# DakeQQ/Audio-Denoiser-ONNX

Measured on AMD Instinct MI355X. Metric: audio_seconds_per_second (GTCRN 16 kHz, batch=256 x 1 s chunks; RTF = 1/value), higher is better.
Workload: dtype f32; 1 GPU; GTCRN 16 kHz, batch=256 x 1 s chunks, fp32, int16 PCM in/out resident in HBM (BASELINE.json configs[1]); chunks_per_gpu=256, chunks_total=256, ranks=1, chunk_samples=16000, out_samples=15872, weights=seeded reference-architecture GTCRN (tests/golden/gtcrn_seed0.adew), stitch_all_gather=False

## Files before the change

### audio_denoiser_onnx_amd/csrc/ade_device.h

```cpp
#pragma once

#include "ade_internal.h"

namespace ade {
namespace dev {

__device__ __forceinline__ float fast_rcp(float x) { return __builtin_amdgcn_rcpf(x); }
__device__ __forceinline__ float fast_sqrt(float x) { return __builtin_amdgcn_sqrtf(x); }
__device__ __forceinline__ float fast_rsq(float x) { return __builtin_amdgcn_rsqf(x); }
__device__ __forceinline__ float sigmoid_f(float x) { return fast_rcp(1.0f + __expf(-x)); }
__device__ __forceinline__ float tanh_f(float x) {
    return 1.0f - 2.0f * fast_rcp(__expf(2.0f * x) + 1.0f);
}
__device__ __forceinline__ float prelu_f(float x, float a) { return x >= 0.0f ? x : a * x; }
__device__ __forceinline__ double shfl_xor_f64(double v, int mask) {
    union { double d; int i[2]; } u;
    u.d = v;
    u.i[0] = __shfl_xor(u.i[0], mask, 64);
    u.i[1] = __shfl_xor(u.i[1], mask, 64);
    return u.d;
}
__device__ __forceinline__ float prelu_sel(float a) { return a <= 1.0f ? __builtin_inff() : -__builtin_inff(); }
__device__ __forceinline__ float prelu_m(float x, float ax, float sel) { return __builtin_amdgcn_fmed3f(x, ax, sel); }

__device__ __forceinline__ void ld4(const float* p, float* v) {
    const float4 q = *reinterpret_cast<const float4*>(p);
    v[0] = q.x; v[1] = q.y; v[2] = q.z; v[3] = q.w;
}
__device__ __forceinline__ void ld8(const float* p, float* v) { ld4(p, v); ld4(p + 4, v + 4); }
__device__ __forceinline__ void ld16(const float* p, float* v) { ld8(p, v); ld8(p + 8, v + 8); }
__device__ __forceinline__ void st4(float* p, const float* v) {
    *reinterpret_cast<float4*>(p) = make_float4(v[0], v[1], v[2], v[3]);
}
__device__ __forceinline__ void st16(float* p, const float* v) { st4(p, v); st4(p + 4, v + 4); st4(p + 8, v + 8); st4(p + 12, v + 12); }

__device__ __forceinline__ void view_ld8_lo(const View& a, size_t pos, size_t frame, float* v) {
    ld8(a.x + pos * kCh, v);
    if (a.at) {
        float g[4];
        ld4(a.at + frame * 8, g);
#pragma unroll
        for (int i = 0; i < 4; ++i) v[2 * i] *= g[i];
    }
}
__device__ __forceinline__ void view_ld8_hi(const View& a, size_t pos, size_t frame, float* v) {
    ld8(a.x + pos * kCh + 8, v);
    if (a.at) {
        float g[4];
        ld4(a.at + frame * 8 + 4, g);
#pragma unroll
        for (int i = 0; i < 4; ++i) v[2 * i] *= g[i];
    }
}
__device__ __forceinline__ void view_ld16(const View& a, size_t pos, size_t frame, float* v) {
    view_ld8_lo(a, pos, frame, v);
    view_ld8_hi(a, pos, frame, v + 8);
}

template <int CTRL>
__device__ __forceinline__ float dpp_mov(float v) {
    return __int_as_float(__builtin_amdgcn_update_dpp(0, __float_as_int(v), CTRL, 0xF, 0xF, true));
}
template <int K> __device__ __forceinline__ float row_bcast(float v) { return dpp_mov<0x150 + K>(v); }
template <int K> __device__ __forceinline__ float quad_bcast(float v) { return dpp_mov<K * 0x55>(v); }
template <int N> __device__ __forceinline__ float row_ror(float v) { return dpp_mov<0x120 + N>(v); }
template <int N> __device__ __forceinline__ float quad_rot(float v) {
    return dpp_mov<((N) & 3) | (((N + 1) & 3) << 2) | (((N + 2) & 3) << 4) | (((N + 3) & 3) << 6)>(v);
}

struct Swapped { float a, b; };
__device__ __forceinline__ Swapped swap16(float v, float s) {
    const auto r = __builtin_amdgcn_permlane16_swap((unsigned)__float_as_int(v), (unsigned)__float_as_int(s), false, false);
    return Swapped{__int_as_float((int)r[0]), __int_as_float((int)r[1])};
}
__device__ __forceinline__ Swapped swap32(float v, float s) {
    const auto r = __builtin_amdgcn_permlane32_swap((unsigned)__float_as_int(v), (unsigned)__float_as_int(s), false, false);
    return Swapped{__int_as_float((int)r[0]), __int_as_float((int)r[1])};
}

template <int LANE> __device__ __forceinline__ float read_lane(float v) {
    return __int_as_float(__builtin_amdgcn_readlane(__float_as_int(v), LANE));
}
constexpr float kLog2e = 1.4426950408889634f;

#if defined(__clang__)
typedef float v4f __attribute__((ext_vector_type(4)));
#else
typedef float v4f __attribute__((vector_size(16)));
#endif
__device__ __forceinline__ v4f mfma16x16x4(float a, float b, v4f c) { return __builtin_amdgcn_mfma_f32_16x16x4f32(a, b, c, 0, 0, 0); }

#if defined(__clang__)
typedef float v2f __attribute__((ext_vector_type(2)));
#else
typedef float v2f __attribute__((vector_size(8)));
#endif
__device__ __forceinline__ v2f mk2(float a, float b) { v2f r; r[0] = a; r[1] = b; return r; }

#if defined(__has_attribute)
#if __has_attribute(address_space)
#define ADE_CONSTANT_AS __attribute__((address_space(4)))
#endif
#endif
#ifndef ADE_CONSTANT_AS
#define ADE_CONSTANT_AS
#endif
#if defined(__AMDGCN__)
#define ADE_KEEP_IN_LOOP(p) asm volatile("" : "+s"(p))
#else
#define ADE_KEEP_IN_LOOP(p) ((void)0)
#endif
#if defined(__AMDGCN__)
#define ADE_KEEP_AFTER(p, tok) asm volatile("" : "+s"(p), "+v"(tok))
#else
#define ADE_KEEP_AFTER(p, tok) ((void)0)
#endif
#if defined(__AMDGCN__)
#define ADE_SCALAR_COPY(dst, src) asm volatile("s_mov_b64 %0, %1" : "=s"(dst) : "s"(src))
#else
#define ADE_SCALAR_COPY(dst, src) ((dst) = (src))
#endif
#if defined(__AMDGCN__)
#define ADE_OPAQUE_V(x) asm volatile("" : "+v"(x))
#else
#define ADE_OPAQUE_V(x) ((void)0)
#endif
template <class T>
__device__ __forceinline__ T cload(const void ADE_CONSTANT_AS* p) {
    static_assert(sizeof(T) % 4 == 0, "dword-sized structs only");
    union U { T v; unsigned w[sizeof(T) / 4]; __device__ U() {} } u;
    const unsigned ADE_CONSTANT_AS* s = (const unsigned ADE_CONSTANT_AS*)p;
#pragma unroll
    for (size_t i = 0; i < sizeof(T) / 4; ++i) u.w[i] = s[i];
    return u.v;
}
typedef const float ADE_CONSTANT_AS* cfptr;
__device__ __forceinline__ cfptr cptr(const float* p) { return (cfptr)p; }

__device__ __forceinline__ void wave_sync() { __builtin_amdgcn_wave_barrier(); }
__device__ __forceinline__ float2 fcmul(float2 a, float2 b) { return make_float2(a.x * b.x - a.y * b.y, a.x * b.y + a.y * b.x); }
__device__ __forceinline__ void fradix4(float2* v) {
    const float2 a0 = make_float2(v[0].x + v[2].x, v[0].y + v[2].y);
    const float2 a1 = make_float2(v[0].x - v[2].x, v[0].y - v[2].y);
    const float2 a2 = make_float2(v[1].x + v[3].x, v[1].y + v[3].y);
    const float2 d = make_float2(v[1].x - v[3].x, v[1].y - v[3].y);
    const float2 a3 = make_float2(d.y, -d.x);
    v[0] = make_float2(a0.x + a2.x, a0.y + a2.y);
    v[1] = make_float2(a1.x + a3.x, a1.y + a3.y);
    v[2] = make_float2(a0.x - a2.x, a0.y - a2.y);
    v[3] = make_float2(a1.x - a3.x, a1.y - a3.y);
}
__device__ __forceinline__ void fft256_inplace(float2* v, float2* buf, int lane, const float2* __restrict__ tw256) {
    fradix4(v);
#pragma unroll
    for (int r = 0; r < 4; ++r) buf[4 * lane + r] = v[r];
    wave_sync();
#pragma unroll
    for (int pass = 1; pass < 4; ++pass) {
        const int Ns = 1 << (2 * pass);
        const int k = lane & (Ns - 1);
        const int tstride = 64 / Ns;
#pragma unroll
        for (int r = 0; r < 4; ++r) v[r] = buf[lane + 64 * r];
#pragma unroll
        for (int r = 1; r < 4; ++r) v[r] = fcmul(v[r], tw256[r * k * tstride]);
        fradix4(v);
        if (pass < 3) {
            wave_sync();
            const int j0 = ((lane - k) << 2) + k;
#pragma unroll
            for (int r = 0; r < 4; ++r) buf[j0 + r * Ns] = v[r];
            wave_sync();
        }
    }
}

__device__ __forceinline__ float4 keep4(bool ok, const float4& v) { return make_float4(ok ? v.x : 0.0f, ok ? v.y : 0.0f, ok ? v.z : 0.0f, ok ? v.w : 0.0f); }
__device__ __attribute__((aligned(16))) static float g_zero4[4] = {0.0f, 0.0f, 0.0f, 0.0f};
__device__ __forceinline__ float4 ld4_or_zero(bool ok, const float* p) { return *reinterpret_cast<const float4*>(ok ? p : g_zero4); }
__device__ __forceinline__ float4 pick4(bool first, const float4& a, const float4& b) {
    return make_float4(first ? a.x : b.x, first ? a.y : b.y, first ? a.z : b.z, first ? a.w : b.w);
}

#if defined(__AMDGCN__)
typedef unsigned ade_v4u __attribute__((ext_vector_type(4)));
__device__ __forceinline__ float4 xld4(const float* base, int float_off) {
    const __amdgpu_buffer_rsrc_t r = __builtin_amdgcn_make_buffer_rsrc(const_cast<float*>(base), 0, 0x7fffffff, 0x00020000);
    const ade_v4u v = __builtin_amdgcn_raw_buffer_load_b128(r, float_off * 4, 0, 16);
    return make_float4(__int_as_float((int)v.x), __int_as_float((int)v.y), __int_as_float((int)v.z), __int_as_float((int)v.w));
}
__device__ __forceinline__ void xst4(float* base, int float_off, const float4& v) {
    const __amdgpu_buffer_rsrc_t r = __builtin_amdgcn_make_buffer_rsrc(base, 0, 0x7fffffff, 0x00020000);
    ade_v4u u;
    u.x = (unsigned)__float_as_int(v.x); u.y = (unsigned)__float_as_int(v.y); u.z = (unsigned)__float_as_int(v.z); u.w = (unsigned)__float_as_int(v.w);
    __builtin_amdgcn_raw_buffer_store_b128(u, r, float_off * 4, 0, 16);
}
__device__ __forceinline__ float xld1(const float* p) { return __hip_atomic_load(p, __ATOMIC_RELAXED, __HIP_MEMORY_SCOPE_AGENT); }
__device__ __forceinline__ void xst1(float* p, float v) { __hip_atomic_store(p, v, __ATOMIC_RELAXED, __HIP_MEMORY_SCOPE_AGENT); }
__device__ __forceinline__ unsigned xflag_load(const unsigned* p) { return __hip_atomic_load(p, __ATOMIC_RELAXED, __HIP_MEMORY_SCOPE_AGENT); }
__device__ __forceinline__ void xflag_store(unsigned* p, unsigned v) { __hip_atomic_store(p, v, __ATOMIC_RELAXED, __HIP_MEMORY_SCOPE_AGENT); }
__device__ __forceinline__ void xdrain() { asm volatile("s_waitcnt vmcnt(0)" ::: "memory"); }
#else
__device__ __forceinline__ float4 xld4(const float* base, int float_off) { return *reinterpret_cast<const float4*>(base + float_off); }
__device__ __forceinline__ void xst4(float* base, int float_off, const float4& v) { *reinterpret_cast<float4*>(base + float_off) = v; }
__device__ __forceinline__ float xld1(const float* p) { return *p; }
__device__ __forceinline__ void xst1(float* p, float v) { *p = v; }
__device__ __forceinline__ unsigned xflag_load(const unsigned* p) { return *(const volatile unsigned*)p; }
__device__ __forceinline__ void xflag_store(unsigned* p, unsigned v) { *(volatile unsigned*)p = v; }
__device__ __forceinline__ void xdrain() {}
#endif
#if defined(__AMDGCN__)
__device__ __forceinline__ int xlimit() {
    const int ADE_CONSTANT_AS* p = (const int ADE_CONSTANT_AS*)__builtin_amdgcn_kernarg_segment_ptr();
    asm volatile("" : "+s"(p));
    return *p;
}
#else
__device__ __forceinline__ int xlimit() { return 20000000; }
#endif
__device__ __forceinline__ int xcode(int flag_index) { return (int)((blockIdx.x + 1u) << 4) | flag_index; }
__device__ __forceinline__ void xwait(unsigned* flag, int* err, int code) {
    if (xflag_load(flag) == 0u) {
        const long long t0 = wall_clock64();
        const int limit = xlimit();
        bool looked = false;
        do {
            __builtin_amdgcn_s_sleep(4);
            const long long dt = wall_clock64() - t0;
            if (dt > (limit >> 4) && !looked) {
                looked = true;
                if (*reinterpret_cast<volatile int*>(err) != 0) return;
            }
            if (dt > limit) {
                volatile int* const e = reinterpret_cast<volatile int*>(err);
                if (*e == 0) *e = code;
                return;
            }
        } while (xflag_load(flag) == 0u);
    }
    xflag_store(flag, 0u);
}

#if defined(__AMDGCN__)
__device__ __forceinline__ unsigned sys_load(const unsigned* p) { return __hip_atomic_load(p, __ATOMIC_RELAXED, __HIP_MEMORY_SCOPE_SYSTEM); }
__device__ __forceinline__ void sys_store(unsigned* p, unsigned v) { __hip_atomic_store(p, v, __ATOMIC_RELAXED, __HIP_MEMORY_SCOPE_SYSTEM); }
__device__ __forceinline__ void sys_acquire() { __builtin_amdgcn_fence(__ATOMIC_ACQUIRE, ""); }
__device__ __forceinline__ void sys_release() { __builtin_amdgcn_fence(__ATOMIC_RELEASE, ""); asm volatile("s_waitcnt vmcnt(0)" ::: "memory"); }
#else
__device__ __forceinline__ unsigned sys_load(const unsigned* p) { return *(const volatile unsigned*)p; }
__device__ __forceinline__ void sys_store(unsigned* p, unsigned v) { *(volatile unsigned*)p = v; }
__device__ __forceinline__ void sys_acquire() {}
__device__ __forceinline__ void sys_release() {}
#endif
__device__ __forceinline__ void wait_rows_in(const unsigned* ready, unsigned epoch, int* err, int code) {
    if (sys_load(ready) != epoch) {
        const long long t0 = wall_clock64();
        const int limit = xlimit();
        do {
            __builtin_amdgcn_s_sleep(8);
            if (wall_clock64() - t0 > limit) {
                volatile int* const e = reinterpret_cast<volatile int*>(err);
                if (*e == 0) *e = code;
                break;
            }
        } while (sys_load(ready) != epoch);
    }
    sys_acquire();
}
__device__ __forceinline__ void signal_rows_out(unsigned* count, unsigned* done, unsigned epoch, unsigned wgs) {
    sys_release();
#if defined(__AMDGCN__)
    const unsigned old = __hip_atomic_fetch_add(count, 1u, __ATOMIC_RELAXED, __HIP_MEMORY_SCOPE_AGENT);
#else
    const unsigned old = (*count)++;
#endif
    if (old + 1u == wgs) {
        xflag_store(count, 0u);
        sys_store(done, epoch);
    }
}

__device__ __forceinline__ void set_prio(int p) {
    if (p == 0) __builtin_amdgcn_s_setprio(0);
    else if (p == 1) __builtin_amdgcn_s_setprio(1);
    else if (p == 2) __builtin_amdgcn_s_setprio(2);
    else __builtin_amdgcn_s_setprio(3);
}

inline dim3 grid1(long long n, int per) { return dim3((unsigned)((n + per - 1) / per)); }

}
}
```

### audio_denoiser_onnx_amd/csrc/ade_engine.hip

```cpp
#include "ade_internal.h"
#include "ade_gtcrn_pack.h"

#include "../../include/ade.h"

#if !defined(HIPSIM)
#include <dlfcn.h>
#endif

#include <algorithm>
#include <cmath>
#include <cstdio>
#include <cstdlib>
#include <cstring>
#include <map>
#include <mutex>
#include <string>
#include <vector>

using namespace ade;

namespace {

thread_local std::string g_create_error;

// ... 311 lines not shown

ade_status build_device_constants(ade_engine* e) {
    Loader L{e};
    Arena A;
    const size_t o_win = A.alloc(kNfft), o_tw256 = A.alloc(512), o_tw512 = A.alloc(2 * 257 + 2), o_ws = A.alloc(kHop);
    {
        const float step = (float)(2.0 * M_PI / (double)kNfft);
        for (int n = 0; n < kNfft; ++n) A.f[o_win + n] = sqrtf(cosf((float)n * step) * -0.5f + 0.5f);
        for (int k = 0; k < 256; ++k) {
            A.f[o_tw256 + 2 * k] = (float)cos(2.0 * M_PI * k / 256.0);
            A.f[o_tw256 + 2 * k + 1] = (float)-sin(2.0 * M_PI * k / 256.0);
        }
        for (int k = 0; k <= 256; ++k) {
            A.f[o_tw512 + 2 * k] = (float)cos(2.0 * M_PI * k / 512.0);
            A.f[o_tw512 + 2 * k + 1] = (float)-sin(2.0 * M_PI * k / 512.0);
        }
        A.f[o_tw512 + 2 * 256] = -1.0f;
        A.f[o_tw512 + 2 * 256 + 1] = 0.0f;
        A.f[o_tw512 + 2 * 128] = 0.0f;
        A.f[o_tw256 + 2 * 64] = 0.0f;
        A.f[o_tw256 + 2 * 128 + 1] = 0.0f;
        A.f[o_tw256 + 2 * 192] = 0.0f;
        for (int r = 0; r < kHop; ++r) {
            const float a = A.f[o_win + r] * A.f[o_win + r], b = A.f[o_win + kHop + r] * A.f[o_win + kHop + r];
            A.f[o_ws + r] = a + b;
        }
    }
    const float* erb_t = L.get("erb.erb_weight_t", {kErbHigh, kErbBands});
    const float* ierb_t = L.get("erb.ierb_weight_t", {kErbBands, kErbHigh});
    if (L.st != ADE_OK) return L.st;
    std::vector<int> bm_start, bs_start;
    std::vector<float> bm_w, bs_w;
    int bm_count = 0, bs_count = 0;
    band_table(erb_t, kErbHigh, kErbBands, bm_start, bm_w, bm_count);
    band_table(ierb_t, kErbBands, kErbHigh, bs_start, bs_w, bs_count);
    const size_t o_bm = A.alloc(bm_w.size()), o_bs = A.alloc(bs_w.size());
    memcpy(&A.f[o_bm], bm_w.data(), bm_w.size() * 4);
    memcpy(&A.f[o_bs], bs_w.data(), bs_w.size() * 4);
    const float* w0 = L.get("encoder.en_convs.0.conv.weight", {16, 9, 1, 5});
    const float* b0 = L.get("encoder.en_convs.0.conv.bias", {16});
    const float* a0 = L.get("encoder.en_convs.0.act.weight", {1});
    const float* w1 = L.get("encoder.en_convs.1.conv.weight", {16, 8, 1, 5});
    const float* b1 = L.get("encoder.en_convs.1.conv.bias", {16});
    const float* a1 = L.get("encoder.en_convs.1.act.weight", {1});
    const float* w3 = L.get("decoder.de_convs.3.conv.weight", {16, 8, 1, 5});
    const float* b3 = L.get("decoder.de_convs.3.conv.bias", {16});
    const float* a3 = L.get("decoder.de_convs.3.act.weight", {1});
    const float* w4 = L.get("decoder.de_convs.4.conv.weight", {16, 2, 1, 5});
    const float* b4 = L.get("decoder.de_convs.4.conv.bias", {2});
    if (L.st != ADE_OK) return L.st;
    const size_t o_w0 = A.alloc(5 * 9 * 16 + 3 * 8 * 16), o_b0 = A.alloc(16), o_w1 = A.alloc(5 * 2 * 8 * 8), o_b1 = A.alloc(16);
    const size_t o_w3 = A.alloc(5 * 2 * 8 * 8), o_b3 = A.alloc(16), o_w4 = A.alloc(5 * 16 * 2), o_b4 = A.alloc(2);
    for (int co = 0; co < 16; ++co)
        for (int ci = 0; ci < 9; ++ci)
            for (int k = 0; k < 5; ++k) A.f[o_w0 + (k * 9 + ci) * 16 + co] = w0[(co * 9 + ci) * 5 + k];
    for (int co = 0; co < 16; ++co)
        for (int c = 0; c < 3; ++c) {
            for (int jj = 0; jj < 7; ++jj) {
                float sum = 0.0f;
                for (int k = 0; k < 5; ++k) {
                    const int o = jj - k;
                    if (o >= 0 && o < 3) sum += w0[(co * 9 + c * 3 + o) * 5 + k];
                }
                A.f[o_w0 + 720 + (c * 8 + jj) * 16 + co] = sum;
            }
            A.f[o_w0 + 720 + (c * 8 + 7) * 16 + co] = -w0[(co * 9 + c * 3 + 2) * 5 + 1];
        }
    for (int g = 0; g < 2; ++g)
        for (int co = 0; co < 8; ++co)
            for (int ci = 0; ci < 8; ++ci)
                for (int k = 0; k < 5; ++k) {
                    A.f[o_w1 + ((k * 2 + g) * 8 + ci) * 8 + co] = w1[((g * 8 + co) * 8 + ci) * 5 + k];
                    A.f[o_w3 + ((k * 2 + g) * 8 + ci) * 8 + co] = w3[((g * 8 + ci) * 8 + co) * 5 + k];
                }
    for (int ci = 0; ci < 16; ++ci)
        for (int co = 0; co < 2; ++co)
            for (int k = 0; k < 5; ++k) A.f[o_w4 + (k * 16 + ci) * 2 + co] = w4[(ci * 2 + co) * 5 + k];
    memcpy(&A.f[o_b0], b0, 64);
    memcpy(&A.f[o_b1], b1, 64);
    memcpy(&A.f[o_b3], b3, 64);
    memcpy(&A.f[o_b4], b4, 8);
    GtOff gte[3], gtd[3];
    DpOff dpo[2];
    static const int en_dil[3] = {1, 2, 5}, de_dil[3] = {5, 2, 1};
    for (int i = 0; i < 3; ++i) {
        if (!load_gt(L, A, "encoder.en_convs." + std::to_string(i + 2) + ".", false, gte[i])) return L.st;
        if (!load_gt(L, A, "decoder.de_convs." + std::to_string(i) + ".", true, gtd[i])) return L.st;
    }
    if (!load_dp(L, A, "dpgrnn1.", dpo[0]) || !load_dp(L, A, "dpgrnn2.", dpo[1])) return L.st;

    HIP_TRY(e, hipMalloc((void**)&e->d_weights, A.f.size() * sizeof(float)));
    HIP_TRY(e, hipMemcpy(e->d_weights, A.f.data(), A.f.size() * sizeof(float), hipMemcpyHostToDevice));
    std::vector<int> ints(bm_start);
    ints.insert(ints.end(), bs_start.begin(), bs_start.end());
    HIP_TRY(e, hipMalloc((void**)&e->d_ints, ints.size() * sizeof(int)));
    HIP_TRY(e, hipMalloc((void**)&e->d_clk, kClkSlots * sizeof(long long)));
    HIP_TRY(e, hipMemset(e->d_clk, 0, kClkSlots * sizeof(long long)));
    HIP_TRY(e, hipMemcpy(e->d_ints, ints.data(), ints.size() * sizeof(int), hipMemcpyHostToDevice));
    const float* W = e->d_weights;
    e->tabs.win = W + o_win;
    e->tabs.tw256 = reinterpret_cast<const float2*>(W + o_tw256);
    e->tabs.tw512 = reinterpret_cast<const float2*>(W + o_tw512);
    e->tabs.win_sum = W + o_ws;
    e->erb_bm = BandTab{e->d_ints, W + o_bm, bm_count, kErbBands};
    e->erb_bs = BandTab{e->d_ints + kErbBands, W + o_bs, bs_count, kErbHigh};
    e->en0 = ConvW{W + o_w0, W + o_b0, a0[0]};
    e->en1 = ConvW{W + o_w1, W + o_b1, a1[0]};
    e->de3 = ConvW{W + o_w3, W + o_b3, a3[0]};
    e->de4 = ConvW{W + o_w4, W + o_b4, 0.0f};
    for (int i = 0; i < 3; ++i) {
        const GtOff* src[2] = {&gte[i], &gtd[i]};
        GtConvW* dst[2] = {&e->en_gt[i], &e->de_gt[i]};
        for (int k = 0; k < 2; ++k) {
            const GtOff& o = *src[k];
            *dst[k] = GtConvW{W + o.pw1, W + o.pw1_b, W + o.dw, W + o.dw_b, W + o.pw2, W + o.pw2_b, W + o.gru, W + o.fc,
                              o.s1, o.s2, k == 0 ? en_dil[i] : de_dil[i], W + o.tra_rot};
        }
    }
    for (int i = 0; i < 2; ++i) {
        const DpOff& o = dpo[i];
        e->dp[i] = DpW{W + o.intra_gru, W + o.inter_gru, W + o.fc[0], W + o.fc_b[0], W + o.ln_w[0], W + o.ln_b[0],
                       W + o.fc[1], W + o.fc_b[1], W + o.ln_w[1], W + o.ln_b[1], W + o.inter_rot};
    }
    return ADE_OK;
}

void free_graphs(ade_engine* e) {
    for (auto& g : e->graphs) {
        if (g.exec) hipGraphExecDestroy(g.exec);
        if (g.graph) hipGraphDestroy(g.graph);
    }
    e->graphs.clear();
}

void free_exchange(ade_engine* e) {
    if (e->d_xchg) hipFree(e->d_xchg);
    if (e->d_xflags) hipFree(e->d_xflags);
    e->d_xchg = nullptr; e->d_xflags = nullptr;
    e->xchg_capacity = 0; e->xchg_segments = 0;
}

void free_workspace(ade_engine* e) {
    free_graphs(e);
    if (e->ws) hipFree(e->ws);
    if (e->d_pcm_in) hipFree(e->d_pcm_in);
    if (e->d_pcm_out) hipFree(e->d_pcm_out);
    if (e->d_f32_out) hipFree(e->d_f32_out);
    if (e->h_pcm_in) hipHostFree(e->h_pcm_in);
    if (e->h_pcm_out) hipHostFree(e->h_pcm_out);
    if (e->h_f32_out) hipHostFree(e->h_f32_out);
    if (e->rs_in) hipFree(e->rs_in);
    if (e->rs_out) hipFree(e->rs_out);
    if (e->d_fixed) hipFree(e->d_fixed);
    e->d_fixed = nullptr;
    free_exchange(e);
    for (float** p : {&e->gt_tmp, &e->gt_in, &e->gt_wave, &e->gt_mean, &e->d_f32_in}) { if (*p) hipFree(*p); *p = nullptr; }
    for (uint16_t** p : {&e->d_f16_in, &e->d_f16_out}) { if (*p) hipFree(*p); *p = nullptr; }
    for (uint16_t** p : {&e->h_f16_in, &e->h_f16_out}) { if (*p) hipHostFree(*p); *p = nullptr; }
    e->f16_capacity = 0;
    e->rs_in = e->rs_out = nullptr;
    e->ws = nullptr;
    e->d_pcm_in = e->d_pcm_out = nullptr;
    e->d_f32_out = nullptr;
    e->h_pcm_in = e->h_pcm_out = nullptr;
    e->h_f32_out = nullptr;
    e->capacity = 0;
}

int pick_geometry(const ade_engine* e, int B);

ade_status ensure_exchange(ade_engine* e) {
    if (e->sub) return ADE_OK;
    if (!e->d_xerr) {
        HIP_TRY(e, hipHostMalloc((void**)&e->d_xerr, kXErrWords * sizeof(int), hipHostMallocDefault));
        for (int k = 0; k < kXErrWords; ++k) e->d_xerr[k] = 0;
    }
    int nseg = 0;
    if (e->use_fused && !e->gt_sand) {
        const int g = pick_geometry(e, e->capacity);
        if (g >= 0) nseg = fused_segments(e->T, g);
    }
    if (nseg <= 1) nseg = 0;
    if (nseg == e->xchg_segments && (nseg == 0 || e->xchg_capacity >= e->capacity)) return ADE_OK;
    if (e->d_xchg && nseg <= e->xchg_segments && e->xchg_capacity >= e->capacity) return ADE_OK;
    if (e->stream) HIP_TRY(e, hipStreamSynchronize(e->stream));
    free_graphs(e);
    free_exchange(e);
    if (nseg) {
        const size_t B = (size_t)e->capacity;
        HIP_TRY(e, hipMalloc((void**)&e->d_xchg, B * nseg * (size_t)kXFloats * sizeof(float)));
        HIP_TRY(e, hipMalloc((void**)&e->d_xflags, B * nseg * (size_t)kXFlags * sizeof(unsigned)));
        HIP_TRY(e, hipMemset(e->d_xflags, 0, B * nseg * (size_t)kXFlags * sizeof(unsigned)));
        e->xchg_capacity = e->capacity;
    }
    e->xchg_segments = nseg;
    return ADE_OK;
}

ade_status reserve(ade_engine* e, int batch) {
    if (batch <= e->capacity) return ensure_exchange(e);
    HIP_TRY(e, hipSetDevice(e->device));
    if (e->stream) HIP_TRY(e, hipStreamSynchronize(e->stream));
    free_workspace(e);
    const size_t B = (size_t)batch, T = (size_t)e->T;
    if (e->sub) {
        std::string derr;
        const int rc = e->sub->reserve(batch, derr);
        if (rc != ADE_OK) return fail(e, (ade_status)rc, derr);
        HIP_TRY(e, hipMalloc((void**)&e->d_pcm_in, B * e->in_len * sizeof(int16_t)));
        HIP_TRY(e, hipMalloc((void**)&e->d_pcm_out, B * e->out_len * sizeof(int16_t)));
        HIP_TRY(e, hipMalloc((void**)&e->d_f32_out, B * e->out_len * sizeof(float)));
        HIP_TRY(e, hipHostMalloc((void**)&e->h_pcm_in, B * e->in_len * sizeof(int16_t), hipHostMallocDefault));
        HIP_TRY(e, hipHostMalloc((void**)&e->h_pcm_out, B * e->out_len * sizeof(int16_t), hipHostMallocDefault));
        HIP_TRY(e, hipHostMalloc((void**)&e->h_f32_out, B * e->out_len * sizeof(float), hipHostMallocDefault));
        if (e->resample) {
            HIP_TRY(e, hipMalloc((void**)&e->rs_in, B * e->channels * e->rs_model_in * sizeof(float)));
            HIP_TRY(e, hipMalloc((void**)&e->rs_out, B * e->out_channels * e->n_outputs * e->rs_model_out * sizeof(float)));
        }
        if (e->gt_float_in) HIP_TRY(e, hipMalloc((void**)&e->d_f32_in, B * (size_t)e->in_len * sizeof(float)));
        e->capacity = batch;
        return ADE_OK;
    }
    const size_t nfr = B * T;
    struct Carve { float** p; size_t n; };
    std::vector<Carve> cs = {
        {&e->mean, B}, {&e->spec, nfr * 2 * kBinsPad}, {&e->feat, nfr * 3 * kErbPad}, {&e->e0, nfr * kF1 * kCh},
        {&e->e1, nfr * kFw * kCh}, {&e->h, nfr * kFw * kCh}, {&e->zt, nfr * 8}, {&e->rnn, nfr * kFw * kCh},
        {&e->d3, nfr * kF1 * kCh}, {&e->mask, nfr * 2 * kErbPad}, {&e->frames, nfr * kNfft}};
    for (int i = 0; i < 3; ++i) {
        cs.push_back({&e->xe[i], nfr * kFw * kCh});
        cs.push_back({&e->ate[i], nfr * 8});
        cs.push_back({&e->xd[i], nfr * kFw * kCh});
        cs.push_back({&e->atd[i], nfr * 8});
    }
    for (int i = 0; i < 2; ++i) {
        cs.push_back({&e->dpm[i], nfr * kFw * kCh});
        cs.push_back({&e->dpo[i], nfr * kFw * kCh});
    }
    size_t total = 0;
    for (auto& c : cs) total += (c.n + 63) & ~(size_t)63;
    HIP_TRY(e, hipMalloc((void**)&e->ws, total * sizeof(float)));
    size_t off = 0;
    for (auto& c : cs) {
        *c.p = e->ws + off;
        off += (c.n + 63) & ~(size_t)63;
    }
    HIP_TRY(e, hipMalloc((void**)&e->d_pcm_in, B * e->in_len * sizeof(int16_t)));
    HIP_TRY(e, hipMalloc((void**)&e->d_pcm_out, B * e->out_len * sizeof(int16_t)));
    HIP_TRY(e, hipMalloc((void**)&e->d_f32_out, B * e->out_len * sizeof(float)));
    HIP_TRY(e, hipHostMalloc((void**)&e->h_pcm_in, B * e->in_len * sizeof(int16_t), hipHostMallocDefault));
    HIP_TRY(e, hipHostMalloc((void**)&e->h_pcm_out, B * e->out_len * sizeof(int16_t), hipHostMallocDefault));
    HIP_TRY(e, hipHostMalloc((void**)&e->h_f32_out, B * e->out_len * sizeof(float), hipHostMallocDefault));
    {
        ChunkFixed F{};
        F.tabs = e->tabs; F.erb_bm = e->erb_bm; F.erb_bs = e->erb_bs;
        F.en0 = e->en0; F.en1 = e->en1; F.de3 = e->de3; F.de4 = e->de4;
        for (int i = 0; i < 3; ++i) { F.en_gt[i] = e->en_gt[i]; F.de_gt[i] = e->de_gt[i]; F.xe[i] = e->xe[i]; F.xd[i] = e->xd[i]; }
        for (int i = 0; i < 2; ++i) { F.dp[i] = e->dp[i]; F.dpo[i] = e->dpo[i]; }
        F.spec = e->spec; F.e0 = e->e0; F.e1 = e->e1;
        HIP_TRY(e, hipMalloc((void**)&e->d_fixed, sizeof(ChunkFixed)));
        HIP_TRY(e, hipMemcpy(e->d_fixed, &F, sizeof(ChunkFixed), hipMemcpyHostToDevice));
    }
    if (e->gt_sand) {
        HIP_TRY(e, hipMalloc((void**)&e->gt_tmp, B * (size_t)e->gt_l1 * sizeof(float)));
        HIP_TRY(e, hipMalloc((void**)&e->gt_in, B * (size_t)e->gt_lm * sizeof(float)));
        HIP_TRY(e, hipMalloc((void**)&e->gt_wave, B * (size_t)e->gt_keep * sizeof(float)));
        HIP_TRY(e, hipMalloc((void**)&e->gt_mean, B * sizeof(float)));
        if (e->gt_float_in) HIP_TRY(e, hipMalloc((void**)&e->d_f32_in, B * (size_t)e->in_len * sizeof(float)));
    }
    e->capacity = batch;
    return ensure_exchange(e);
}

struct Seq {
    ade_engine* e;
    hipStream_t s;
    bool prof;
    int cursor = 0;
    void begin(const char* name) {
        if (!prof) return;
        int si = -1;
        for (size_t i = 0; i < e->stats.size(); ++i)
            if (e->stats[i].name == name) si = (int)i;
        if (si < 0) { e->stats.push_back(KernelStat{name, 0.f, 0}); si = (int)e->stats.size() - 1; }
        if ((int)e->events.size() <= cursor) {
            hipEvent_t a, b;
            hipEventCreate(&a);
            hipEventCreate(&b);
            e->events.push_back({a, b});
            e->event_stat.push_back(si);
        }
        e->event_stat[cursor] = si;
        hipEventRecord(e->events[cursor].first, s);
    }
    void end() {
        if (!prof) return;
        hipEventRecord(e->events[cursor].second, s);
        ++cursor;
        e->events_used = cursor;
    }
};

int pick_geometry(const ade_engine* e, int ) {
    if (e->geometry >= 0) return fused_supported(e->T, e->geometry) ? e->geometry : -1;
    for (int g = fused_geometries() - 1; g >= 0; --g)
        if (fused_supported(e->T, g)) return g;
    return -1;
}

void enqueue(ade_engine* e, hipStream_t s, const int16_t* d_in, int B, int16_t* d_out, float* d_f32, bool prof) {
    const int T = e->T, nfr = B * T;
    Seq q{e, s, prof};
    const View none{nullptr, nullptr};
    const int geo = pick_geometry(e, B);
    const bool fused = e->use_fused && geo >= 0 && !e->gt_sand;
    e->last_fused = fused;
    View x{e->e1, nullptr};
    if (fused) {
        SegPlan plan{};
        plan.nseg = fused_segments(T, geo); plan.xchg = e->d_xchg; plan.flags = e->d_xflags; plan.err = e->d_xerr; plan.wave_swap = e->wave_swap;
        plan.prio = e->seg_prio;
        plan.withhold = e->xchg_withhold;
        plan.wait_ticks = e->xwait_ticks;
        e->last_geometry = geo;
        long long* clk = prof ? e->d_clk : nullptr;
        if (clk) (void)hipMemsetAsync(e->d_clk, 0, kClkSlots * sizeof(long long), s);
        const float* dc = nullptr;
        if (e->n_win > 1) {
            q.begin("pcm_mean"); launch_pcm_mean(s, d_in, B, e->in_len, e->mean, e->n_win); q.end();
            dc = e->mean;
        }
        if (e->use_single && (!prof || e->profile_mode >= 2)) {
            ChunkCall C{};
            C.fixed = e->d_fixed;
            C.dc = dc;
            C.stagger = (geo == 0 && B >= 192) ? e->stagger_ticks : 0;
            C.pcm_in = d_in; C.pcm_out = d_out; C.f32_out = d_f32; C.L = e->in_len; C.T = T; C.B = B;
            C.plan = plan;
            C.full_taps = e->full_taps;
            C.clk = (prof && e->profile_mode == 3) ? e->d_clk : nullptr;
            q.begin("gtcrn_chunk"); launch_gtcrn_chunk(s, geo, C); q.end();
            return;
        }
        q.begin("front"); launch_front(s, geo, plan, d_in, B, e->in_len, T, e->tabs, e->erb_bm, e->en0, e->en1, e->spec, e->e0, e->e1, clk, dc); q.end();
        for (int i = 0; i < 3; ++i) {
            q.begin("gtblock"); launch_gtblock(s, geo, plan, i, x.x, nullptr, e->en_gt[i], e->xe[i], B, T, (prof && i == 0) ? e->d_clk : nullptr); q.end();
            x = View{e->xe[i], nullptr};
        }
        for (int i = 0; i < 2; ++i) {
            q.begin("dpgrnn"); launch_dpgrnn(s, geo, plan, i, x.x, e->dp[i], e->dpo[i], B, T, (prof && i == 0) ? e->d_clk : nullptr); q.end();
            x = View{e->dpo[i], nullptr};
        }
        for (int i = 0; i < 3; ++i) {
            q.begin("gtblock"); launch_gtblock(s, geo, plan, 3 + i, x.x, e->xe[2 - i], e->de_gt[i], e->xd[i], B, T, nullptr); q.end();
            x = View{e->xd[i], nullptr};
        }
        q.begin("back"); launch_back(s, geo, plan, x.x, e->e1, e->e0, e->spec, e->de3, e->de4, e->erb_bs, e->tabs, d_out, d_f32, B, T, clk); q.end();
        return;
    }
    if (e->gt_sand) {
        q.begin("sandwich_in");
        launch_gt_sandwich_in(s, e->cur_fin ? nullptr : d_in, e->cur_fin, B / e->n_win, e->in_len * e->n_win, e->gt_l1 * e->n_win, e->gt_lm * e->n_win, e->gt_lerp1,
                              e->gt_lerp2, e->gt_gain, e->gt_tmp, e->gt_mean, e->gt_in);
        q.end();
        q.begin("stft_feat"); launch_stft_pcm(s, nullptr, nullptr, B, e->gt_lm, T, e->tabs, e->erb_bm, e->spec, e->feat, true, e->gt_in); q.end();
    } else {
        q.begin("pcm_mean"); launch_pcm_mean(s, d_in, B, e->in_len, e->mean, e->n_win); q.end();
        q.begin("stft_feat"); launch_stft_pcm(s, d_in, e->mean, B, e->in_len, T, e->tabs, e->erb_bm, e->spec, e->feat); q.end();
    }
    q.begin("conv0"); launch_conv0(s, e->feat, e->en0, e->e0, nfr); q.end();
    q.begin("conv1"); launch_conv1(s, e->e0, e->en1, e->e1, nfr); q.end();
    for (int i = 0; i < 3; ++i) {
        q.begin("gt_pw1"); launch_gt_pw1(s, x, none, e->en_gt[i], e->h, nfr); q.end();
        q.begin("gt_dw_pw2"); launch_gt_dw_pw2(s, e->h, x, none, e->en_gt[i], e->xe[i], e->zt, B, T); q.end();
        q.begin("tra_gru"); launch_tra(s, e->zt, e->en_gt[i], e->ate[i], B, T); q.end();
        x = View{e->xe[i], e->ate[i]};
    }
    for (int i = 0; i < 2; ++i) {
        q.begin("intra_gru"); launch_intra_gru(s, x, e->dp[i].intra_gru, e->rnn, nfr); q.end();
        q.begin("fc_ln_res"); launch_fc_ln_res(s, e->rnn, x, e->dp[i].intra_fc, e->dp[i].intra_fc_b, e->dp[i].intra_ln_w,
                                               e->dp[i].intra_ln_b, e->dpm[i], B, T); q.end();
        q.begin("inter_gru"); launch_inter_gru(s, e->dpm[i], e->dp[i].inter_gru, e->rnn, B, T, nullptr, e->dp[i].inter_rot); q.end();
        q.begin("fc_ln_res"); launch_fc_ln_res(s, e->rnn, View{e->dpm[i], nullptr}, e->dp[i].inter_fc, e->dp[i].inter_fc_b,
                                               e->dp[i].inter_ln_w, e->dp[i].inter_ln_b, e->dpo[i], B, T); q.end();
        x = View{e->dpo[i], nullptr};
    }
    for (int i = 0; i < 3; ++i) {
        const View skip{e->xe[2 - i], e->ate[2 - i]};
        q.begin("gt_pw1"); launch_gt_pw1(s, x, skip, e->de_gt[i], e->h, nfr); q.end();
        q.begin("gt_dw_pw2"); launch_gt_dw_pw2(s, e->h, x, skip, e->de_gt[i], e->xd[i], e->zt, B, T); q.end();
        q.begin("tra_gru"); launch_tra(s, e->zt, e->de_gt[i], e->atd[i], B, T); q.end();
        x = View{e->xd[i], e->atd[i]};
    }
    q.begin("deconv3"); launch_deconv3(s, x, View{e->e1, nullptr}, e->de3, e->d3, nfr); q.end();
    q.begin("deconv4"); launch_deconv4(s, e->d3, e->e0, e->de4, e->mask, nfr); q.end();
    q.begin("istft_mask"); launch_istft_masked(s, e->spec, e->mask, e->erb_bs, e->tabs, e->frames, nfr); q.end();
    if (e->gt_sand) {
        q.begin("sandwich_out");
        launch_gt_sandwich_out(s, e->frames, e->tabs, B, T, e->gt_keep, e->gt_wave, d_out, d_f32, e->out_len, e->gt_lerp_out, e->gt_scale_first);
        q.end();
        return;
    }
    q.begin("ola_pcm"); launch_ola_pcm(s, e->frames, e->tabs, B, T, d_out, d_f32); q.end();
}

ade_status run(ade_engine* e, hipStream_t s, const int16_t* d_in, int B, int16_t* d_out, float* d_f32) {
    if (B == 0) return ADE_OK;
    e->last_batch = B;
    std::string sub_err;
    int sub_rc = ADE_OK;
    auto launch_all = [&](bool timed) {
        if (e->sub && e->resample) {
            const long long rows_in = (long long)B * e->channels, rows_out = (long long)B * e->out_channels * e->n_outputs;
            if (e->cur_fin) launch_resample_in_f32(s, e->cur_fin, e->rs_in, rows_in, e->in_len / e->channels, e->rs_model_in, e->rs_scale_in, e->rs_in_gain);
            else launch_resample_in(s, d_in, e->rs_in, rows_in, e->in_len / e->channels, e->rs_model_in, e->rs_scale_in);
            e->sub->float_in = e->rs_in;
            e->sub->float_src = e->cur_fin;
            e->sub->float_src_gain = e->rs_in_gain;
            sub_rc = e->sub->run(s, d_in, B, nullptr, e->rs_out, sub_err);
            e->sub->float_in = nullptr;
            e->sub->float_src = nullptr;
            if (e->rs_sandwich_out)
                launch_gt_out(s, e->rs_out, d_out, d_f32, rows_out, e->rs_model_out, e->out_len / (e->out_channels * e->n_outputs), e->rs_scale_out, e->rs_scale_first,
                              e->rs_nan_to_num);
            else
                launch_resample_out(s, e->rs_out, d_out, d_f32, rows_out, e->rs_model_out, e->out_len / (e->out_channels * e->n_outputs), e->rs_scale_out,
                                    e->rs_pcm_scale, e->rs_truncate_i32, e->rs_f32_scale, e->rs_nan_to_num);
        } else if (e->sub) sub_rc = e->sub->run(s, d_in, B, d_out, d_f32, sub_err);
        else enqueue(e, s, d_in, B, d_out, d_f32, timed);
    };
    if (e->sub && (e->profile || !e->use_graph || !e->graph_supported)) {
        launch_all(false);
        return sub_rc == ADE_OK ? ADE_OK : fail(e, (ade_status)sub_rc, sub_err);
    }
    if (e->profile) {
        for (auto& st : e->stats) { st.ms = 0.f; st.launches = 0; }
        e->events_used = 0;
        enqueue(e, s, d_in, B, d_out, d_f32, true);
        HIP_TRY(e, hipStreamSynchronize(s));
        for (size_t i = 0; i < (size_t)e->events_used; ++i) {
            float ms = 0.f;
            hipEventElapsedTime(&ms, e->events[i].first, e->events[i].second);
            e->stats[e->event_stat[i]].ms += ms;
            e->stats[e->event_stat[i]].launches += 1;
        }
        return ADE_OK;
    }
    const bool one_kernel = !e->sub && e->use_fused && e->use_single && pick_geometry(e, B) >= 0 && !e->gt_sand;
    if (e->use_graph && e->graph_supported && !one_kernel) {
        GraphEntry* hit = nullptr;
        for (auto& g : e->graphs)
            if (g.in == d_in && g.out_pcm == d_out && g.out_f32 == d_f32 && g.batch == B) hit = &g;
        if (!hit) {
            if (hipStreamBeginCapture(s, hipStreamCaptureModeThreadLocal) == hipSuccess) {
                launch_all(false);
                hipGraph_t graph = nullptr;
                hipGraphExec_t exec = nullptr;
                if (hipStreamEndCapture(s, &graph) == hipSuccess && graph && sub_rc == ADE_OK &&
                    hipGraphInstantiate(&exec, graph, nullptr, nullptr, 0) == hipSuccess) {
                    if (e->graphs.size() >= 8) {
                        hipGraphExecDestroy(e->graphs.front().exec);
                        hipGraphDestroy(e->graphs.front().graph);
                        e->graphs.erase(e->graphs.begin());
                    }
                    e->graphs.push_back(GraphEntry{d_in, d_out, d_f32, B, exec, graph});
                    hit = &e->graphs.back();
                } else {
                    if (graph) hipGraphDestroy(graph);
                    e->graph_supported = false;
                }
            } else {
                (void)hipGetLastError();
                e->graph_supported = false;
            }
        }
        if (hit) {
            HIP_TRY(e, hipGraphLaunch(hit->exec, s));
            return ADE_OK;
        }
    }
    launch_all(false);
    if (sub_rc != ADE_OK) return fail(e, (ade_status)sub_rc, sub_err);
    HIP_TRY(e, hipGetLastError());
    return ADE_OK;
}

const char* xflag_name(int idx) {
    return idx < kXFlagTra ? "depthwise-convolution history" : (idx < kXFlagInter ? "TRA state" : (idx < kXFlagOla ? "inter-frame GRU state" : "overlap-add carry"));
}
ade_status exchange_status(ade_engine* h, const char* who, bool earlier) {
    if (h->sub) {
        const int code = h->sub->exchange_error_and_reset();
        if (code) {
            h->timed_out = true;
            char msg[320];
            snprintf(msg, sizeof msg, "%s: %s: a segment hand-off (%s) of the fused network stages timed out (%.1f ms)%s; the call's output is not valid "
                     "(ADE_HG_FUSED=0 runs the multi-kernel sequence, option xwait_ms raises the bound)", who, "sub-engine", xflag_name(code & 15), h->xwait_ticks * 1e-5,
                     earlier ? " in an earlier call on a caller-provided stream" : "");
            return fail(h, ADE_ERR_DEVICE, msg);
        }
    }
    if (!h->d_xerr) return ADE_OK;
    int code = 0, word = 0;
    for (int k = 0; k < kXErrWords && !code; ++k) { code = ((volatile int*)h->d_xerr)[k]; word = k; }
    if (!code) return ADE_OK;
    (void)hipDeviceSynchronize();
    for (int k = 0; k < kXErrWords; ++k) h->d_xerr[k] = 0;
    if (h->d_xflags) (void)hipMemset(h->d_xflags, 0, (size_t)h->xchg_capacity * h->xchg_segments * kXFlags * sizeof(unsigned));
    const int block = (code >> 4) - 1, idx = code & 15, B = h->xl_B[word] > 0 ? h->xl_B[word] : (h->last_batch > 0 ? h->last_batch : 1), chunk0 = h->xl_B[word] > 0 ? h->xl_chunk0[word] : 0;
    h->timed_out = true;
    char msg[384];
    if (idx == 15)
        snprintf(msg, sizeof msg, "%s: fused path%s: segment %d of chunk %d timed out (%.1f ms) waiting for its rows of the host batch to be copied in; no output was produced "
                 "(option host_stream=1 copies the batch before the launch, option xwait_ms raises the bound)",
                 who, earlier ? " (an earlier call on a caller-provided stream)" : "", block / B, chunk0 + block % B, h->xwait_ticks * 1e-5);
    else
        snprintf(msg, sizeof msg,
                 "%s: fused path%s: segment %d of chunk %d timed out (%.1f ms) waiting for the %s of its predecessor workgroup; no output was produced "
                 "(option geometry=0 runs whole chunks per workgroup, option xwait_ms raises the bound)",
                 who, earlier ? " (an earlier call on a caller-provided stream)" : "", block / B, chunk0 + block % B, h->xwait_ticks * 1e-5, xflag_name(idx));
    return fail(h, ADE_ERR_DEVICE, msg);
}

}

struct ade_stream {
    ade_engine* e = nullptr;
    int device = 0;
    int S = 0, N = 0;
    bool first = true, flushed = false;
    void* sub_state = nullptr;
    int in_ch = 1, delay = kHop;
    int16_t *pcm_prev = nullptr, *pcm_hist = nullptr, *concat = nullptr, *d_in = nullptr, *d_out = nullptr, *h_in = nullptr, *h_out = nullptr;
    float *d_f32 = nullptr, *h_f32 = nullptr;
    float* state = nullptr;
    size_t state_floats = 0;
    float* dc = nullptr;
    float* hist[6][2] = {};
    int hist_cur[6] = {};
    float* tra_h[6] = {};
    float* inter_h[2] = {};
    float* carry = nullptr;
    bool fused = false;
    int geo = -1, geo_flush = -1;
    ade::ChunkFixed* d_fixed = nullptr;
    float* xq = nullptr;
    unsigned* xq_flags = nullptr;
    float* xstate[2] = {};
    unsigned* xstate_flags[2] = {};
    int xcur = 0;
    int* xerr = nullptr;
    float* ws = nullptr;
    float *spec = nullptr, *feat = nullptr, *e0 = nullptr, *e1 = nullptr, *h = nullptr, *zt = nullptr, *rnn = nullptr, *d3 = nullptr, *mask = nullptr,
          *frames = nullptr, *xe[3] = {}, *ate[3] = {}, *xd[3] = {}, *atd[3] = {}, *dpm[2] = {}, *dpo[2] = {};
};

namespace {

void enqueue_stream(ade_stream* st, hipStream_t s, const int16_t* d_in, int16_t* d_out, float* d_f32, bool flush = false) {
    ade_engine* e = st->e;
    const int B = st->S, T = flush ? 1 : st->N, nfr = B * T, P = T * kHop;
    if (flush) launch_stream_concat_flush(s, st->pcm_hist, st->pcm_prev, st->concat, B);
    else {
        launch_stream_concat(s, st->pcm_hist, d_in, st->concat, B, P, st->first);
        launch_stream_keep(s, st->concat, st->pcm_hist, st->pcm_prev, B, P);
    }
    if (st->fused) {
        const int geo = flush ? st->geo_flush : st->geo;
        ChunkCall C{};
        C.fixed = st->d_fixed;
        C.pcm_in = st->concat; C.pcm_out = d_out; C.f32_out = d_f32; C.dc = st->dc;
        C.L = P + kHop; C.T = T; C.B = B;
        SegPlan plan{};
        plan.nseg = fused_segments(T, geo);
        plan.xchg = st->xq; plan.flags = st->xq_flags; plan.err = st->xerr;
        plan.wait_ticks = e->xwait_ticks;
        plan.carry_in = st->first ? nullptr : st->xstate[st->xcur];
        plan.carry_in_flags = st->first ? nullptr : st->xstate_flags[st->xcur];
        plan.carry_out = st->xstate[st->xcur ^ 1];
        plan.carry_out_flags = st->xstate_flags[st->xcur ^ 1];
        plan.stream = 1;
        C.plan = plan;
        launch_gtcrn_chunk(s, geo, C);
        st->xcur ^= 1;
        st->first = false;
        return;
    }
    launch_stft_pcm(s, st->concat, st->dc, B, P + kHop, T, e->tabs, e->erb_bm, st->spec, st->feat, false);
    launch_conv0(s, st->feat, e->en0, st->e0, nfr);
    launch_conv1(s, st->e0, e->en1, st->e1, nfr);
    const View none{nullptr, nullptr};
    View x{st->e1, nullptr};
    auto gt_block = [&](int gi, const GtConvW& w, View in, View skip, float* xn, float* at) {
        launch_gt_pw1(s, in, skip, w, st->h, nfr);
        const int cur = st->hist_cur[gi];
        launch_gt_dw_pw2(s, st->h, in, skip, w, xn, st->zt, B, T, st->hist[gi][cur]);
        launch_hist_shift(s, st->hist[gi][cur], st->h, st->hist[gi][cur ^ 1], B, T, 2 * w.dilation);
        st->hist_cur[gi] = cur ^ 1;
        launch_tra(s, st->zt, w, at, B, T, st->tra_h[gi]);
    };
    for (int i = 0; i < 3; ++i) {
        gt_block(i, e->en_gt[i], x, none, st->xe[i], st->ate[i]);
        x = View{st->xe[i], st->ate[i]};
    }
    for (int i = 0; i < 2; ++i) {
        launch_intra_gru(s, x, e->dp[i].intra_gru, st->rnn, nfr);
// ... 1465 lines not shown
```

### audio_denoiser_onnx_amd/csrc/ade_stage_frontback.h

```cpp
#pragma once
#include "ade_stage_net.h"

namespace ade {
namespace stage {

constexpr int kWbuf = 264;
constexpr size_t kTabFloats = 512 + 2 * 256 + 2 * 264;
constexpr int kBmCap = 16;
constexpr int kBsCap = 4;

__device__ __forceinline__ float2 rfft_bin(float2 zk, float2 zp, float2 w) {
    const float2 e = make_float2(0.5f * (zk.x + zp.x), 0.5f * (zk.y - zp.y));
    const float2 d = make_float2(0.5f * (zk.x - zp.x), 0.5f * (zk.y + zp.y));
    const float2 o = make_float2(d.y, -d.x);
    return make_float2(e.x + (w.x * o.x - w.y * o.y), e.y + (w.x * o.y + w.y * o.x));
}

struct LdsTabs { const float* win; const float2* tw256; const float2* tw512; };
template <class G>
__device__ __forceinline__ LdsTabs stage_tables(float* dst, const FftTabs& t, int tid) {
    constexpr int kFusedThreads = G::kThreads;
    float* win = dst;
    float* tw256 = dst + 512;
    float* tw512 = tw256 + 512;
    for (int i = tid; i < 512; i += kFusedThreads) { win[i] = t.win[i]; tw256[i] = reinterpret_cast<const float*>(t.tw256)[i]; }
    for (int i = tid; i < 514; i += kFusedThreads) tw512[i] = reinterpret_cast<const float*>(t.tw512)[i];
    return LdsTabs{win, reinterpret_cast<const float2*>(tw256), reinterpret_cast<const float2*>(tw512)};
}

__device__ __forceinline__ void load_frame_pairs(const int16_t* __restrict__ row, int L, int t, int lane, bool live, bool pair_ok, int* raw, int centre = kNfft / 2) {
#pragma unroll
    for (int r = 0; r < 4; ++r) {
        const int n = lane + 64 * r;
        const int j0 = kHop * t + 2 * n - centre;
        if (!live) {
            raw[r] = 0;
        } else if (pair_ok && j0 >= 0 && j0 + 1 < L) {
            raw[r] = *reinterpret_cast<const int*>(row + j0);
        } else {
            int ja = j0, jb = j0 + 1;
            ja = ja < 0 ? -ja : (ja >= L ? 2 * (L - 1) - ja : ja);
            jb = jb < 0 ? -jb : (jb >= L ? 2 * (L - 1) - jb : jb);
            raw[r] = ((int)row[ja] & 0xffff) | ((int)row[jb] << 16);
        }
    }
}

__device__ __forceinline__ void erb_merge(const float* wtab, int count, int s0, const float2* buf, int lane, float* fr) {
    float a0 = 0.0f, a1 = 0.0f, a2 = 0.0f;
    for (int n = 0; n < count; ++n) {
        const float wv = wtab[n * kErbBands + lane];
        const float2 x = buf[kErbLow + min(s0 + n, kErbHigh - 1)];
        a0 += fast_sqrt((x.x * x.x + x.y * x.y) + 1e-12f) * wv;
        a1 += x.x * wv;
        a2 += x.y * wv;
    }
    fr[kErbLow + lane] = a0;
    fr[kErb + kErbLow + lane] = a1;
    fr[2 * kErb + kErbLow + lane] = a2;
}

constexpr int kC0TailW = 27 * 16;
constexpr int kC1TailW = 3 * 2 * 64;
template <class G> constexpr size_t front_smem_bytes() {
    return ((size_t)G::kTileF * kWbuf * 2 + (size_t)G::kTileF * 3 * kErb + (size_t)4 * G::kTileF * kF1 * 4 + kTabFloats +
            (size_t)(G::kLean ? 0 : kBmCap) * kErbBands + kC0TailW + kC1TailW + 16) * 4;
}

template <class G>
__device__ __forceinline__ void front_stage(float* smem, int chunk, const Seg& sg, const int16_t* __restrict__ pcm, int L, const FftTabs& tabs,
                                            const BandTab& erb, const ConvW& c0, const ConvW& c1, float* __restrict__ spec,
                                            float* __restrict__ e0, float* __restrict__ e1, long long* __restrict__ clk,
                                            const float* __restrict__ dc_rows = nullptr) {
    constexpr int kFusedThreads = G::kThreads, kTileF = G::kTileF, kTileP1 = kTileF * kF1;
    constexpr size_t kFrontFeatFloats = (size_t)kTileF * 3 * kErb;
    constexpr int kGroupShift = (kFusedThreads == 1024 ? 9 : (kFusedThreads == 512 ? 8 : 7));
    static_assert(kFusedThreads == 1024 || kFusedThreads == 512 || kFusedThreads == 256, "front / back conv rounds: 64 lanes per frame");
    constexpr int kBmRows = G::kLean ? 0 : kBmCap;
    const int T = sg.T, tbeg = sg.t0, tend = sg.t0 + sg.nT;
    float2* wbuf_all = reinterpret_cast<float2*>(smem);
    float* feat = smem + kTileF * kWbuf * 2;
    float4* E0 = reinterpret_cast<float4*>(feat + kFrontFeatFloats);
    float* E0f = reinterpret_cast<float*>(E0);
    float* tabmem = reinterpret_cast<float*>(E0 + 4 * kTileP1);
    float* erbw = tabmem + kTabFloats;
    float* w0t = erbw + kBmRows * kErbBands;
    float* w1t = w0t + kC0TailW;
    int* red = reinterpret_cast<int*>(w1t + kC1TailW);
    int tid_ = threadIdx.x;
    ADE_OPAQUE_V(tid_);
    const int tid = tid_, wave = tid >> 6, lane = tid & 63;
    const int16_t* row = pcm + (size_t)chunk * L;
    const int P0 = T * kF1, P = T * kFw;
    float* e0c = e0 + (size_t)chunk * kCh * P0;
    float* e1c = e1 + (size_t)chunk * kCh * P;
    float* specc = spec + (size_t)chunk * T * 2 * kBinsPad;
    ADE_CLK(32);
    const bool pair_ok = ((L & 1) == 0) && ((reinterpret_cast<size_t>(row) & 3) == 0);
    int raw[4];
    const int centre = sg.stream ? 0 : kNfft / 2;
    load_frame_pairs(row, L, tbeg + wave, lane, tbeg + wave < tend, pair_ok, raw, centre);
    const LdsTabs lt = stage_tables<G>(tabmem, tabs, tid);
    const bool erb_lds = erb.count <= kBmRows;
    if (erb_lds)
        for (int i = tid; i < erb.count * kErbBands; i += kFusedThreads) erbw[i] = erb.w[i];
    const int erb_s0 = erb.start[lane];
    for (int i = tid; i < kC0TailW; i += kFusedThreads) w0t[i] = c0.w[i];
    for (int i = tid; i < kC1TailW; i += kFusedThreads) w1t[i] = c1.w[i];
    const float b0t = c0.b[tid & 15], b1t = c1.b[tid & 15];

    if (!dc_rows) {
        int s = 0;
        if (((L & 7) == 0) && ((reinterpret_cast<size_t>(row) & 15) == 0)) {
            const int4* r4 = reinterpret_cast<const int4*>(row);
#pragma unroll 2
            for (int i = tid; i < (L >> 3); i += kFusedThreads) {
                const int4 q = r4[i];
                s += (int)(short)(q.x & 0xffff) + (q.x >> 16) + (int)(short)(q.y & 0xffff) + (q.y >> 16)
                   + (int)(short)(q.z & 0xffff) + (q.z >> 16) + (int)(short)(q.w & 0xffff) + (q.w >> 16);
            }
        } else {
            for (int i = tid; i < L; i += kFusedThreads) s += (int)row[i];
        }
#pragma unroll
        for (int off = 32; off >= 1; off >>= 1) s += __shfl_xor(s, off);
        if (lane == 0) red[wave] = s;
    }
    __syncthreads();
    float dc;
    if (dc_rows) {
        dc = dc_rows[chunk];
    } else {
        long long tot = 0;
#pragma unroll
        for (int i = 0; i < kTileF; ++i) tot += red[i];
        dc = (float)((double)tot / ((double)L * 32768.0));
    }
    ADE_CLK(33);
    long long clk_prev = ADE_CLK_START();
    const cfptr c0b = cptr(c0.b), c1b = cptr(c1.b);
    const cfptr c0e = cptr(c0.w) + 5 * 9 * 16;

    for (int t0 = tbeg; t0 < tend; t0 += kTileF) {
        const int nf = tend - t0 < kTileF ? tend - t0 : kTileF;
        {
            int tq = tid;
            ADE_OPAQUE_V(tq);
            const int wave = tq >> 6, lane = tq & 63;
            float2* buf = wbuf_all + wave * kWbuf;
            const int t = t0 + wave;
            const bool live = wave < nf;
            float2 v[4];
#pragma unroll
            for (int r = 0; r < 4; ++r) {
                const int n = lane + 64 * r;
                const float sa = (float)(short)(raw[r] & 0xffff) * (1.0f / 32768.0f) - dc;
                const float sb = (float)(raw[r] >> 16) * (1.0f / 32768.0f) - dc;
                v[r] = make_float2(sa * lt.win[2 * n], sb * lt.win[2 * n + 1]);
            }
            {
                const int tn = t + kTileF;
                load_frame_pairs(row, L, tn, lane, tn < tend, pair_ok, raw, centre);
            }
            fft256_inplace(v, buf, lane, lt.tw256);
            wave_sync();
#pragma unroll
            for (int r = 0; r < 4; ++r) buf[lane + 64 * r] = v[r];
            wave_sync();
            {
                float2 xa[2], xb[2];
#pragma unroll
                for (int r = 0; r < 2; ++r) {
                    const int k = lane + 64 * r;
                    const float2 zk = buf[k], zp = buf[(256 - k) & 255];
                    xa[r] = rfft_bin(zk, zp, lt.tw512[k]);
                    xb[r] = rfft_bin(zp, zk, lt.tw512[256 - k]);
                }
                float2 xm = make_float2(0.0f, 0.0f);
                if (lane == 0) { const float2 z = buf[128]; xm = rfft_bin(z, z, lt.tw512[128]); }
                wave_sync();
#pragma unroll
                for (int r = 0; r < 2; ++r) {
                    const int k = lane + 64 * r;
                    buf[k] = xa[r];
                    buf[256 - k] = xb[r];
                }
                if (lane == 0) buf[128] = xm;
            }
            wave_sync();
            if (live) {
                float* fr = feat + (size_t)wave * 3 * kErb;
#pragma unroll
                for (int r = 0; r < 5; ++r) {
                    if (r == 4 && lane != 0) break;
                    const int k = r < 4 ? lane + 64 * r : 256;
                    const float2 x = buf[k];
                    specc[((size_t)t * 2 + 0) * kBinsPad + k] = x.x;
                    specc[((size_t)t * 2 + 1) * kBinsPad + k] = x.y;
                    if (k < kErbLow) {
                        fr[k] = fast_sqrt((x.x * x.x + x.y * x.y) + 1e-12f);
                        fr[kErb + k] = x.x;
                        fr[2 * kErb + k] = x.y;
                    }
                }
                if (erb_lds) erb_merge(erbw, erb.count, erb_s0, buf, lane, fr);
                else erb_merge(erb.w, erb.count, erb_s0, buf, lane, fr);
            }
        }
        __syncthreads();
        ADE_CLK(34);
        ADE_CLK_ACC(40);
        {
            int tq = tid;
            ADE_OPAQUE_V(tq);
            const int tl = tq >> 6, g = (tq >> 4) & 3, j = tq & 15;
            if (tl < nf) {
                const float* fr = feat + (size_t)tl * 3 * kErb;
                float wa[6];
#pragma unroll
                for (int kk = 0; kk < 6; ++kk) wa[kk] = c0e[((kk >> 1) * 8 + 4 * (kk & 1) + g) * 16 + j];
                v4f cb;
#pragma unroll
                for (int r = 0; r < 4; ++r) cb[r] = c0b[4 * g + r];
                const float sel0 = prelu_sel(c0.slope);
#pragma unroll
                for (int mt = 0; mt < 4; ++mt) {
                    const int fo = 16 * mt + j;
                    const int q0 = 2 * fo - 3 + g;
                    const bool v0 = q0 >= 0;
                    const int q1 = g == 3 ? 0 : 2 * fo + 1 + g;
                    const bool v1 = g == 3 ? fo == 0 : q1 < kErb;
                    v4f d = cb;
#pragma unroll
                    for (int c = 0; c < 3; ++c) {
                        const float x0 = fr[c * kErb + q0], x1 = fr[c * kErb + q1];
                        d = mfma16x16x4(wa[2 * c], v0 ? x0 : 0.0f, d);
                        d = mfma16x16x4(wa[2 * c + 1], v1 ? x1 : 0.0f, d);
                    }
                    const float4 r4 = make_float4(prelu_m(d[0], d[0] * c0.slope, sel0), prelu_m(d[1], d[1] * c0.slope, sel0),
                                                  prelu_m(d[2], d[2] * c0.slope, sel0), prelu_m(d[3], d[3] * c0.slope, sel0));
                    const int idx = tl * kF1 + fo;
                    E0[g * kTileP1 + idx] = r4;
                    *reinterpret_cast<float4*>(e0c + ((size_t)g * P0 + (size_t)t0 * kF1 + idx) * 4) = r4;
                }
            }
        }
        if (tid < kTileF * 16) {
            int tq = tid;
            ADE_OPAQUE_V(tq);
            const int tl = tq >> 4, co = tq & 15;
            if (tl < nf) {
                const float* fr = feat + (size_t)tl * 3 * kErb;
                float acc = b0t;
#pragma unroll
                for (int k = 0; k < 3; ++k)
#pragma unroll
                    for (int c = 0; c < 3; ++c)
#pragma unroll
                        for (int o = 0; o < 3; ++o) {
                            const int q = 2 * (kF1 - 1) - 3 + k + o;
                            const float x = q < kErb ? fr[c * kErb + q] : 0.0f;
                            acc += w0t[(k * 9 + c * 3 + o) * 16 + co] * x;
                        }
                acc = prelu_f(acc, c0.slope);
                const int idx = tl * kF1 + (kF1 - 1);
                E0f[((size_t)(co >> 2) * kTileP1 + idx) * 4 + (co & 3)] = acc;
                e0c[((size_t)(co >> 2) * P0 + t0 * kF1 + idx) * 4 + (co & 3)] = acc;
            }
        }
        __syncthreads();
        ADE_CLK(35);
        ADE_CLK_ACC(41);
        {
            int tq = tid;
            ADE_OPAQUE_V(tq);
            const int g = __builtin_amdgcn_readfirstlane(tq >> kGroupShift);
            const int tl = (tq >> 5) & (kTileF - 1), fo = tq & 31;
            if (tl < nf) {
                cfptr cw = cptr(c1.w);
                ADE_KEEP_IN_LOOP(cw);
                float acc[8];
#pragma unroll
                for (int co = 0; co < 8; ++co) acc[co] = c1b[g * 8 + co];
#pragma unroll
                for (int k = 0; k < 5; ++k) {
                    const int fi = 2 * fo - 2 + k;
                    const bool ok = fi >= 0;
                    const int pp = tl * kF1 + (ok ? fi : 0);
                    const float4 xa = E0[(2 * g) * kTileP1 + pp], xb = E0[(2 * g + 1) * kTileP1 + pp];
                    const float x[8] = {ok ? xa.x : 0.0f, ok ? xa.y : 0.0f, ok ? xa.z : 0.0f, ok ? xa.w : 0.0f,
                                        ok ? xb.x : 0.0f, ok ? xb.y : 0.0f, ok ? xb.z : 0.0f, ok ? xb.w : 0.0f};
#pragma unroll
                    for (int ci = 0; ci < 8; ++ci)
#pragma unroll
                        for (int co = 0; co < 8; ++co) acc[co] += cw[((k * 2 + g) * 8 + ci) * 8 + co] * x[ci];
                }
#pragma unroll
                for (int co = 0; co < 8; ++co) acc[co] = prelu_f(acc[co], c1.slope);
                const int p = t0 * kFw + tl * kFw + fo;
                st4(e1c + ((size_t)(2 * g) * P + p) * 4, acc);
                st4(e1c + ((size_t)(2 * g + 1) * P + p) * 4, acc + 4);
            }
        }
        if (tid < kTileF * 16) {
            int tq = tid;
            ADE_OPAQUE_V(tq);
            const int tl = tq >> 4, g = (tq >> 3) & 1, co = tq & 7;
            if (tl < nf) {
                float acc = b1t;
#pragma unroll
                for (int k = 0; k < 3; ++k) {
                    const int pp = tl * kF1 + (kF1 - 3) + k;
#pragma unroll
                    for (int ci = 0; ci < 8; ++ci)
                        acc += w1t[((k * 2 + g) * 8 + ci) * 8 + co] * E0f[((size_t)(2 * g + (ci >> 2)) * kTileP1 + pp) * 4 + (ci & 3)];
                }
                acc = prelu_f(acc, c1.slope);
                const int p = t0 * kFw + tl * kFw + (kFw - 1);
                e1c[((size_t)(2 * g + (co >> 2)) * P + p) * 4 + (co & 3)] = acc;
            }
        }
        ADE_CLK(36);
        ADE_CLK_ACC(42);
    }
}

constexpr int kC3TailW = 2 * 2 * 64;
constexpr int kC4TailW = 2 * 16 * 2;
template <class G> constexpr size_t back_smem_bytes() {
    return ((size_t)4 * G::kTileF * kFw * 4 + (size_t)4 * G::kTileF * kF1 * 4 + (size_t)G::kTileF * 2 * kErbPad + (size_t)kHop + kTabFloats + (size_t)kBsCap * kErbHigh +
            kC3TailW + kC4TailW + (G::kLean ? 0 : kHop + kErbHigh + kHop)) * 4;
}

template <class G>
__device__ __forceinline__ void back_stage(float* smem, int chunk, const Seg& sg, const float* __restrict__ x, const float* __restrict__ e1,
                                           const float* __restrict__ e0, const float* __restrict__ spec, const ConvW& c3, const ConvW& c4,
                                           const BandTab& bs, const FftTabs& tabs, int16_t* __restrict__ pcm,
                                           float* __restrict__ f32, long long* __restrict__ clk) {
    constexpr int kFusedThreads = G::kThreads, kTileF = G::kTileF, kTileP1 = kTileF * kF1, kTileP = kTileF * kFw;
    constexpr size_t kBackAccFloats = (size_t)kNfft + (size_t)kHop * (kTileF - 1);
    static_assert((size_t)4 * kTileP * 4 >= (size_t)kTileF * kWbuf * 2, "the S tile must be able to hold the FFT buffers");
    static_assert((size_t)4 * kTileP1 * 4 >= kBackAccFloats, "the D tile must be able to hold the overlap-add accumulator");
    constexpr int kSUnits = 4 * kTileP;
    constexpr int kSThreads = kSUnits / 3;
    static_assert(kSThreads * 3 == kSUnits && kSThreads <= kFusedThreads, "S staging split");
    constexpr int kGroupShift = (kFusedThreads == 1024 ? 9 : (kFusedThreads == 512 ? 8 : 7));
    constexpr bool kLean = G::kLean;
    const int T = sg.T, tbeg = sg.t0, tend = sg.t0 + sg.nT;
    float4* S = reinterpret_cast<float4*>(smem);
    float* Sf = smem;
    float2* wbuf_all = reinterpret_cast<float2*>(smem);
    float4* D = S + 4 * kTileP;
    float* Df = reinterpret_cast<float*>(D);
    float* M = reinterpret_cast<float*>(D + 4 * kTileP1);
    float* acc = Df;
    float* cbuf = M + kTileF * 2 * kErbPad;
    float* tabmem = cbuf + kHop;
    float* bsw = tabmem + kTabFloats;
    float* w3t = bsw + kBsCap * kErbHigh;
    float* w4t = w3t + kC3TailW;
    float* wsum = kLean ? const_cast<float*>(tabs.win_sum) : w4t + kC4TailW;
    int* bss = reinterpret_cast<int*>(wsum + kHop);
    float* pend = kLean ? sg.xo + kXPendOff : reinterpret_cast<float*>(bss + kErbHigh);
    int tid_ = threadIdx.x;
    ADE_OPAQUE_V(tid_);
    const int tid = tid_;
    const int P0 = T * kF1, P = T * kFw;
    const float* xc = x + (size_t)chunk * kCh * P;
    const float* e1c = e1 + (size_t)chunk * kCh * P;
    const float* e0c = e0 + (size_t)chunk * kCh * P0;
    const float* specc = spec + (size_t)chunk * T * 2 * kBinsPad;
    const int trim = sg.stream ? 0 : kHop;
    const int out_len = sg.stream ? kHop * T : kHop * (T - 1);
    int16_t* po = pcm ? pcm + (size_t)chunk * out_len : nullptr;
    float* fo32 = f32 ? f32 + (size_t)chunk * out_len : nullptr;
    ADE_CLK(48);

    auto issue_s = [&](int t0n, bool go, float4* sa, float4* sb) {
        const int nfn = tend - t0n < kTileF ? tend - t0n : kTileF;
        int tq = tid;
        ADE_OPAQUE_V(tq);
        const bool on = go && tq < kSThreads;
#pragma unroll
        for (int i = 0; i < 3; ++i) {
            const int u = tq + kSThreads * i, q = u / kTileP, idx = u - q * kTileP;
            const int idc = idx < nfn * kFw ? idx : 0;
            const size_t off = ((size_t)q * P + (size_t)t0n * kFw + idc) * 4;
            sa[i] = on ? *reinterpret_cast<const float4*>(xc + off) : make_float4(0.0f, 0.0f, 0.0f, 0.0f);
            sb[i] = on ? *reinterpret_cast<const float4*>(e1c + off) : make_float4(0.0f, 0.0f, 0.0f, 0.0f);
        }
    };
    auto commit_s = [&](const float4* sa, const float4* sb) {
        int tq = tid;
        ADE_OPAQUE_V(tq);
        if (tq < kSThreads) {
#pragma unroll
            for (int i = 0; i < 3; ++i)
                S[tq + kSThreads * i] = make_float4(sa[i].x + sb[i].x, sa[i].y + sb[i].y, sa[i].z + sb[i].z, sa[i].w + sb[i].w);
        }
    };
    auto issue_e0 = [&](int t0n, bool go, float4* ea, float4* eb) {
        const int nfn = tend - t0n < kTileF ? tend - t0n : kTileF;
        int tq = tid;
        ADE_OPAQUE_V(tq);
        const int g = tq >> kGroupShift, tl = (tq >> 5) & (kTileF - 1), m = tq & 31;
        const bool on = go && tl < nfn;
        const int pe = on ? tl * kF1 + 2 * m : 0;
#pragma unroll
        for (int h = 0; h < 2; ++h) {
            const float* src = e0c + ((size_t)(2 * g + h) * P0 + (size_t)t0n * kF1 + pe) * 4;
            ea[h] = on ? *reinterpret_cast<const float4*>(src) : make_float4(0.0f, 0.0f, 0.0f, 0.0f);
            eb[h] = on ? *reinterpret_cast<const float4*>(src + 4) : make_float4(0.0f, 0.0f, 0.0f, 0.0f);
        }
    };
    float4 sa0[3], sb0[3];
    issue_s(tbeg, true, sa0, sb0);
    float4 ea[2], eb[2];
    issue_e0(tbeg, true, ea, eb);
    const LdsTabs lt = stage_tables<G>(tabmem, tabs, tid);
    if (!kLean)
        for (int i = tid; i < kHop; i += kFusedThreads) wsum[i] = tabs.win_sum[i];
    const bool bs_lds = bs.count <= kBsCap;
    int bs_s[4] = {0, 0, 0, 0};
    if (bs_lds) {
        for (int i = tid; i < bs.count * kErbHigh; i += kFusedThreads) bsw[i] = bs.w[i];
        if (!kLean) {
            for (int i = tid; i < kErbHigh; i += kFusedThreads) bss[i] = bs.start[i];
        } else {
            int tq = tid;
            ADE_OPAQUE_V(tq);
            const int lane = tq & 63;
#pragma unroll
            for (int r = 1; r < 5; ++r) {
                const int k = r < 4 ? lane + 64 * r : 256;
                bs_s[r - 1] = (k >= kErbLow && (r < 4 || lane == 0)) ? bs.start[k - kErbLow] : 0;
            }
        }
    }
    for (int i = tid; i < kC3TailW; i += kFusedThreads) w3t[i] = c3.w[(i < 128 ? 2 : 4) * 128 + (i & 127)];
    for (int i = tid; i < kC4TailW; i += kFusedThreads) w4t[i] = c4.w[(i < 32 ? 2 : 4) * 32 + (i & 31)];
    const float b3t = c3.b[tid & 15], b4t = c4.b[tid & 1];
    for (int i = tid; i < kHop; i += kFusedThreads) cbuf[i] = 0.0f;
    const cfptr c3b = cptr(c3.b), c4b = cptr(c4.b), c4w = cptr(c4.w);
    commit_s(sa0, sb0);
    long long clk_prev = ADE_CLK_START();

    for (int t0 = tbeg; t0 < tend; t0 += kTileF) {
        const int nf = tend - t0 < kTileF ? tend - t0 : kTileF;
        float sre[5], sim[5];
        float wsr[4] = {1.0f, 1.0f, 1.0f, 1.0f};
        if (kLean) ld4(wsum + ((tid * 4) & (kHop - 1)), wsr);
        {
            int tq = tid;
            ADE_OPAQUE_V(tq);
            const int wave = tq >> 6, lane = tq & 63;
            const int tcp = wave < nf ? t0 + wave : t0;
#pragma unroll
            for (int r = 0; r < 5; ++r) {
                const int k = r < 4 ? lane + 64 * r : 256;
                sre[r] = (r < 4 || lane == 0) ? specc[((size_t)tcp * 2 + 0) * kBinsPad + k] : 0.0f;
                sim[r] = (r < 4 || lane == 0) ? specc[((size_t)tcp * 2 + 1) * kBinsPad + k] : 0.0f;
            }
        }
        __syncthreads();
        ADE_CLK(49);
        ADE_CLK_ACC(56);
        {
            int tq = tid;
            ADE_OPAQUE_V(tq);
            const int g = __builtin_amdgcn_readfirstlane(tq >> kGroupShift);
            const int tl = (tq >> 5) & (kTileF - 1), m = tq & 31;
            if (tl < nf) {
                const int idx = tl * kFw + m, pe = tl * kF1 + 2 * m;
                cfptr cw = cptr(c3.w);
                ADE_KEEP_IN_LOOP(cw);
                float ev[8], od[8];
#pragma unroll
                for (int co = 0; co < 8; ++co) { ev[co] = c3b[g * 8 + co]; od[co] = c3b[g * 8 + co]; }
#pragma unroll
                for (int dlt = -1; dlt <= 1; ++dlt) {
                    const bool ok = m + dlt >= 0;
                    const int ke = 2 - 2 * dlt, ko = 3 - 2 * dlt;
                    const int ps = idx + (ok ? dlt : 0);
                    const float4 xa = S[(2 * g) * kTileP + ps], xb = S[(2 * g + 1) * kTileP + ps];
                    const float xv[8] = {ok ? xa.x : 0.0f, ok ? xa.y : 0.0f, ok ? xa.z : 0.0f, ok ? xa.w : 0.0f,
                                         ok ? xb.x : 0.0f, ok ? xb.y : 0.0f, ok ? xb.z : 0.0f, ok ? xb.w : 0.0f};
#pragma unroll
                    for (int ci = 0; ci < 8; ++ci)
#pragma unroll
                        for (int co = 0; co < 8; ++co) {
                            ev[co] += cw[((ke * 2 + g) * 8 + ci) * 8 + co] * xv[ci];
                            if (dlt >= 0) od[co] += cw[((ko * 2 + g) * 8 + ci) * 8 + co] * xv[ci];
                        }
                }
#pragma unroll
                for (int h = 0; h < 2; ++h) {
                    D[(2 * g + h) * kTileP1 + pe] =
                        make_float4(prelu_f(ev[4 * h], c3.slope) + ea[h].x, prelu_f(ev[4 * h + 1], c3.slope) + ea[h].y,
                                    prelu_f(ev[4 * h + 2], c3.slope) + ea[h].z, prelu_f(ev[4 * h + 3], c3.slope) + ea[h].w);
                    D[(2 * g + h) * kTileP1 + pe + 1] =
                        make_float4(prelu_f(od[4 * h], c3.slope) + eb[h].x, prelu_f(od[4 * h + 1], c3.slope) + eb[h].y,
                                    prelu_f(od[4 * h + 2], c3.slope) + eb[h].z, prelu_f(od[4 * h + 3], c3.slope) + eb[h].w);
                }
            }
        }
        if (tid < kTileF * 16) {
            int tq = tid;
            ADE_OPAQUE_V(tq);
            const int tl = tq >> 4, g = (tq >> 3) & 1, co = tq & 7;
            if (tl < nf) {
                const int pe = tl * kF1 + (kF1 - 1);
                const float eadd = e0c[((size_t)(2 * g + (co >> 2)) * P0 + (size_t)t0 * kF1 + pe) * 4 + (co & 3)];
                float ev = b3t;
#pragma unroll
                for (int dlt = -1; dlt <= 0; ++dlt) {
                    const int ps = tl * kFw + (kFw - 1) + dlt;
#pragma unroll
                    for (int ci = 0; ci < 8; ++ci)
                        ev += w3t[(dlt < 0 ? 128 : 0) + (g * 8 + ci) * 8 + co] * Sf[((size_t)(2 * g + (ci >> 2)) * kTileP + ps) * 4 + (ci & 3)];
                }
                Df[((size_t)(2 * g + (co >> 2)) * kTileP1 + pe) * 4 + (co & 3)] = prelu_f(ev, c3.slope) + eadd;
            }
        }
        __syncthreads();
        ADE_CLK(50);
        ADE_CLK_ACC(57);
        float4 sa[3], sb[3];
        const bool has_next = t0 + kTileF < tend;
        issue_s(has_next ? t0 + kTileF : t0, has_next, sa, sb);
        issue_e0(has_next ? t0 + kTileF : t0, has_next, ea, eb);
        {
            int tq = tid;
            ADE_OPAQUE_V(tq);
            const int tl = tq >> 6, m = tq & 63;
            if (tl < nf) {
                const int idx = tl * kF1 + m;
                v2f ev = mk2(c4b[0], c4b[1]), od = ev;
#pragma unroll
                for (int dlt = -1; dlt <= 1; ++dlt) {
                    const bool ok = m + dlt >= 0;
                    const int ke = 2 - 2 * dlt, ko = 3 - 2 * dlt;
#pragma unroll
                    for (int q = 0; q < 4; ++q) {
                        const float4 xq = D[q * kTileP1 + idx + (ok ? dlt : 0)];
                        const float xv[4] = {ok ? xq.x : 0.0f, ok ? xq.y : 0.0f, ok ? xq.z : 0.0f, ok ? xq.w : 0.0f};
#pragma unroll
                        for (int c = 0; c < 4; ++c) {
                            ev += mk2(c4w[(ke * 16 + 4 * q + c) * 2], c4w[(ke * 16 + 4 * q + c) * 2 + 1]) * xv[c];
                            if (dlt >= 0) od += mk2(c4w[(ko * 16 + 4 * q + c) * 2], c4w[(ko * 16 + 4 * q + c) * 2 + 1]) * xv[c];
                        }
                    }
                }
                float* mr = M + (size_t)tl * 2 * kErbPad;
#pragma unroll
                for (int co = 0; co < 2; ++co) {
                    mr[co * kErbPad + 2 * m] = tanh_f(ev[co]);
                    mr[co * kErbPad + 2 * m + 1] = tanh_f(od[co]);
                }
            }
        }
        if (tid < kTileF * 2) {
            const int tl = tid >> 1, co = tid & 1;
            if (tl < nf) {
                float ev = b4t;
#pragma unroll
                for (int dlt = -1; dlt <= 0; ++dlt) {
                    const int ps = tl * kF1 + (kF1 - 1) + dlt;
#pragma unroll
                    for (int ci = 0; ci < 16; ++ci)
                        ev += w4t[(dlt < 0 ? 32 : 0) + ci * 2 + co] * Df[((size_t)(ci >> 2) * kTileP1 + ps) * 4 + (ci & 3)];
                }
                M[(size_t)tl * 2 * kErbPad + co * kErbPad + (kErb - 1)] = tanh_f(ev);
            }
        }
        __syncthreads();
        ADE_CLK(51);
        ADE_CLK_ACC(58);
        {
            int tq = tid;
            ADE_OPAQUE_V(tq);
            const int wave = tq >> 6, lane = tq & 63;
            float2* buf = wbuf_all + wave * kWbuf;
            const bool live = wave < nf;
            const float* mr = M + (size_t)(live ? wave : 0) * 2 * kErbPad;
#pragma unroll
            for (int r = 0; r < 5; ++r) {
                if (r == 4 && lane != 0) break;
                const int k = r < 4 ? lane + 64 * r : 256;
                const float xr = sre[r], xi = sim[r];
                float m0, m1;
                if (k < kErbLow) {
                    m0 = mr[k];
                    m1 = mr[kErbPad + k];
                } else {
                    const int o = k - kErbLow;
                    m0 = 0.0f; m1 = 0.0f;
                    if (bs_lds) {
                        const int s0 = kLean ? bs_s[r > 0 ? r - 1 : 0] : bss[o];
                        for (int n = 0; n < bs.count; ++n) {
                            const float wv = bsw[n * kErbHigh + o];
                            const int jj = min(s0 + n, kErbBands - 1);
                            m0 += mr[kErbLow + jj] * wv;
                            m1 += mr[kErbPad + kErbLow + jj] * wv;
                        }
                    } else {
                        const int s0 = bs.start[o];
                        for (int n = 0; n < bs.count; ++n) {
                            const float wv = bs.w[n * kErbHigh + o];
                            const int jj = min(s0 + n, kErbBands - 1);
                            m0 += mr[kErbLow + jj] * wv;
                            m1 += mr[kErbPad + kErbLow + jj] * wv;
                        }
                    }
                }
                float2 y = make_float2(__fmaf_rn(xr, m0, -(xi * m1)), __fmaf_rn(xi, m0, xr * m1));
                if (k == 0 || k == 256) y.y = 0.0f;
                buf[k] = y;
            }
            wave_sync();
            float2 v[4];
#pragma unroll
            for (int r = 0; r < 4; ++r) {
                const int k = lane + 64 * r;
                const float2 yk = buf[k], yp = buf[256 - k];
                const float2 e = make_float2(0.5f * (yk.x + yp.x), 0.5f * (yk.y - yp.y));
                const float2 d = make_float2(0.5f * (yk.x - yp.x), 0.5f * (yk.y + yp.y));
                const float2 o = fcmul(d, make_float2(lt.tw512[k].x, -lt.tw512[k].y));
                v[r] = make_float2(e.x - o.y, -(e.y + o.x));
            }
            wave_sync();
            fft256_inplace(v, buf, lane, lt.tw256);
            const bool park = sg.prev && t0 == tbeg && wave == 0;
#pragma unroll
            for (int par = 0; par < 2; ++par) {
                if (live && (wave & 1) == par) {
#pragma unroll
                    for (int r = 0; r < 4; ++r) {
                        const int n = lane + 64 * r;
                        const float pa = v[r].x * (1.0f / 256.0f), pb = -v[r].y * (1.0f / 256.0f);
                        float wa = pa * lt.win[2 * n], wb = pb * lt.win[2 * n + 1];
                        ADE_OPAQUE_V(wa);
                        ADE_OPAQUE_V(wb);
                        float2* a = reinterpret_cast<float2*>(acc + kHop * wave + 2 * n);
                        if (park && r < 2) {
                            *reinterpret_cast<float2*>(pend + 2 * n) = make_float2(wa, wb);
                        } else if (par == 0) {
                            float2 c = make_float2(0.0f, 0.0f);
                            if (wave == 0 && r < 2) c = *reinterpret_cast<const float2*>(cbuf + 2 * n);
                            *a = make_float2(c.x + wa, c.y + wb);
                        } else if (r < 2 || wave + 1 < nf) {
                            float2 c = *a;
                            c.x += wa;
                            c.y += wb;
                            *a = c;
                        } else {
                            *a = make_float2(0.0f + wa, 0.0f + wb);
                        }
                    }
                }
                __syncthreads();
            }
        }
        ADE_CLK(52);
        ADE_CLK_ACC(59);
        if (has_next) commit_s(sa, sb);
        int tf = tid;
        ADE_OPAQUE_V(tf);
        for (int i4 = tf; i4 < nf * (kHop / 4); i4 += kFusedThreads) {
            const int i = i4 * 4;
            const int n = kHop * t0 + i - trim;
            if (n < 0 || n >= out_len) continue;
            float v[4], ws[4];
            ld4(acc + i, v);
            if (sg.stream && sg.first && t0 == 0 && i < kHop) { v[0] = 0.0f; v[1] = 0.0f; v[2] = 0.0f; v[3] = 0.0f; }
            if (sg.prev && t0 == tbeg && i < kHop) continue;
            if (kLean) { ws[0] = wsr[0]; ws[1] = wsr[1]; ws[2] = wsr[2]; ws[3] = wsr[3]; }
            else ld4(wsum + (i & (kHop - 1)), ws);
#pragma unroll
            for (int u = 0; u < 4; ++u) v[u] = v[u] * fast_rcp(ws[u]);
            if (fo32) st4(fo32 + n, v);
            if (po) {
                short q[4];
#pragma unroll
                for (int u = 0; u < 4; ++u) q[u] = (short)(int)fminf(fmaxf(v[u] * 32767.0f, -32768.0f), 32767.0f);
                *reinterpret_cast<short4*>(po + n) = make_short4(q[0], q[1], q[2], q[3]);
            }
        }
        ADE_CLK_ACC(60);
        {
            float carry = 0.0f;
            if (tf < kHop) carry = acc[kHop * nf + tf];
            if (sg.next && !has_next && tf < kHop) xst1(sg.xo + kXOlaOff + tf, carry);
            if (tf < kHop) cbuf[tf] = carry;
        }
        ADE_CLK_ACC(61);
    }
    if (sg.next) {
        xdrain();
        __syncthreads();
        if (tid == 0) xflag_store(sg.fo + kXFlagOla, 1u);
    }
    if (sg.prev) {
        if (tid == 0) xwait(sg.fi + kXFlagOla, sg.err, xcode(kXFlagOla));
        __syncthreads();
        int tf = tid;
        ADE_OPAQUE_V(tf);
        for (int i4 = tf; i4 < kHop / 4; i4 += kFusedThreads) {
            const int i = i4 * 4;
            const int n = kHop * tbeg + i - trim;
            float v[4], ws[4];
            ld4(pend + i, v);
            ld4(wsum + i, ws);
#pragma unroll
            for (int u = 0; u < 4; ++u) v[u] = (xld1(sg.xi + kXOlaOff + i + u) + v[u]) * fast_rcp(ws[u]);
            if (fo32) st4(fo32 + n, v);
            if (po) {
                short q[4];
#pragma unroll
                for (int u = 0; u < 4; ++u) q[u] = (short)(int)fminf(fmaxf(v[u] * 32767.0f, -32768.0f), 32767.0f);
                *reinterpret_cast<short4*>(po + n) = make_short4(q[0], q[1], q[2], q[3]);
            }
        }
    }
    ADE_CLK(53);
}

}
}
```

### audio_denoiser_onnx_amd/csrc/ade_stage_net.h

```cpp
#pragma once
#include "ade_device.h"

#include <type_traits>

#ifndef ADE_DP_INTER_MFMA
#define ADE_DP_INTER_MFMA 0
#endif

namespace ade {
namespace stage {

using namespace dev;


template <int NT, int TMAX, int WAVES_PER_SIMD>
struct Geo {
    static constexpr int kThreads = NT;
    static constexpr int kWavesPerSimd = WAVES_PER_SIMD;
    static constexpr int kTmax = TMAX;
    static constexpr int kPmax = TMAX * kFw;
    static constexpr int kPosPerThread = (kPmax + NT - 1) / NT;
    static constexpr int kTileF = NT / 64;
    static constexpr int kProdBase = ((TMAX * (kFw / 3) + 63) / 64) * 64;
    static constexpr bool kLean = NT < 512;
    static_assert(kPosPerThread == 3, "the conv phases are written for three positions per lane");
    static_assert(kProdBase < NT, "the history producers need a wavefront outside the conv lanes");
};
typedef Geo<1024, 64, 4> Geo0;
typedef Geo<512, 32, 4> Geo1;
typedef Geo<256, 16, 4> Geo2;

__device__ __forceinline__ float comp(const float4& v, int c) { return c == 0 ? v.x : (c == 1 ? v.y : (c == 2 ? v.z : v.w)); }

__device__ __forceinline__ void pl_ld8(const float* Xc, int P, int p, int q0, float* v) {
    ld4(Xc + ((size_t)q0 * P + p) * 4, v);
    ld4(Xc + ((size_t)(q0 + 1) * P + p) * 4, v + 4);
}
__device__ __forceinline__ void pl_ld16(const float* Xc, int P, int p, float* v) {
    pl_ld8(Xc, P, p, 0, v);
    pl_ld8(Xc, P, p, 2, v + 8);
}
__device__ __forceinline__ void pl_st16(float* Xc, int P, int p, const float* v) {
#pragma unroll
    for (int q = 0; q < 4; ++q) st4(Xc + ((size_t)q * P + p) * 4, v + 4 * q);
}

template <class G> constexpr size_t gt_smem_bytes() { return (size_t)4 * G::kPmax * 16 + 2 * G::kTmax * 8 * 4; }

#define ADE_REP16(M) M(0) M(1) M(2) M(3) M(4) M(5) M(6) M(7) M(8) M(9) M(10) M(11) M(12) M(13) M(14) M(15)

#define ADE_CLK(i) do { if (clk && chunk == 0 && threadIdx.x == 0) clk[i] = wall_clock64(); } while (0)
#define ADE_CLK_START() ((clk && chunk == 0 && threadIdx.x == 0) ? wall_clock64() : 0)
#define ADE_CLK_ACC(i) do { if (clk && chunk == 0 && threadIdx.x == 0) { const long long n_ = wall_clock64(); clk[i] += n_ - clk_prev; clk_prev = n_; } } while (0)

template <class G>
__device__ __forceinline__ void gtblock_stage(float4* smem, int chunk, const Seg& sg, int blk, const float* __restrict__ a, const float* __restrict__ skip,
                                              const GtConvW& w, float* __restrict__ out, long long* __restrict__ clk,
                                              bool x1_in_lds = false, bool next_x1 = false, const float* __restrict__ next_skip = nullptr, bool store_lo = true,
                                              bool next_full = false) {
    constexpr int kFusedThreads = G::kThreads, kTmaxFused = G::kTmax, kPmax = G::kPmax, kPosPerThread = G::kPosPerThread;
    float4* H = smem;
    float* zt = reinterpret_cast<float*>(smem + 4 * kPmax);
    float* at = zt + kTmaxFused * 8;
    float* GI = reinterpret_cast<float*>(smem + 2 * kPmax);
    float* HS = GI + kTmaxFused * 48;
    const int T = sg.nT;
    const int P = T * kFw;
    const int Ps = sg.T * kFw;
    int tid_ = threadIdx.x;
    if (kFusedThreads == 512 && sg.swap) tid_ ^= (tid_ & 256) >> 1;
    ADE_OPAQUE_V(tid_);
    const int tid = tid_;
    const size_t cbase = (size_t)chunk * kCh * Ps + (size_t)sg.t0 * kFw * 4;
    const float* ac = a + cbase;
    const float* sc = skip ? skip + cbase : nullptr;
    float* oc = out + cbase;
    const cfptr c_pw1_b = cptr(w.pw1_b), c_dw_b = cptr(w.dw_b), c_pw2_b = cptr(w.pw2_b);
    cfptr c_pw1, c_dw, c_pw2;
    ADE_SCALAR_COPY(c_pw1, cptr(w.pw1));
    ADE_SCALAR_COPY(c_dw, cptr(w.dw));
    ADE_SCALAR_COPY(c_pw2, cptr(w.pw2));
    const float pw1_slope = w.pw1_slope, dw_slope = w.dw_slope;
    const float pw1_sel = prelu_sel(pw1_slope), dw_sel = prelu_sel(dw_slope);
    const int dilation = w.dilation;
    ADE_CLK(0);

    if (!x1_in_lds) {
        constexpr int kIt = (kPmax + kFusedThreads - 1) / kFusedThreads;
        float x[kIt][8], y[kIt][8];
#pragma unroll
        for (int i = 0; i < kIt; ++i) {
            const int p = tid + i * kFusedThreads, pc = p < P ? p : P - 1;
            pl_ld8(ac, Ps, pc, 0, x[i]);
            if (sc) pl_ld8(sc, Ps, pc, 0, y[i]);
        }
#pragma unroll
        for (int i = 0; i < kIt; ++i) {
            const int p = tid + i * kFusedThreads;
            if (p >= P) break;
            if (sc) {
#pragma unroll
                for (int k = 0; k < 8; ++k) x[i][k] += y[i][k];
            }
            H[2 * kPmax + p] = make_float4(x[i][0], x[i][1], x[i][2], x[i][3]);
            H[3 * kPmax + p] = make_float4(x[i][4], x[i][5], x[i][6], x[i][7]);
        }
        __syncthreads();
    }
    constexpr int kWaves = kFusedThreads / 64;
    constexpr int kTiles = (kPmax / 16 + kWaves - 1) / kWaves;
    static_assert(kPmax % 16 == 0, "whole tiles");
    const int wave = __builtin_amdgcn_readfirstlane(tid >> 6);
    const int g = (tid >> 4) & 3, jn = tid & 15;
    const float* Hf = reinterpret_cast<const float*>(H);
    const char* const Hb = reinterpret_cast<const char*>(H);
    constexpr int kZ0 = 4 * kPmax * 16;
    constexpr int kPairs = (kTiles + 1) / 2;
    float4 hi[kPairs];
    {
        float wa[2][6];
#pragma unroll
        for (int kk = 0; kk < 6; ++kk) {
            wa[0][kk] = c_pw1[((4 * (kk & 1) + g) * 3 + (kk >> 1)) * 16 + jn];
            wa[1][kk] = c_pw1[((4 * (kk & 1) + g) * 3 + (kk >> 1)) * 16 + (jn ^ 8)];
        }
        v4f cb[2];
#pragma unroll
        for (int r = 0; r < 4; ++r) { cb[0][r] = c_pw1_b[4 * g + r]; cb[1][r] = c_pw1_b[(4 * g + r) ^ 8]; }
#pragma unroll
        for (int it = 0; it < kTiles; ++it) {
            const int od = it & 1;
            const int pu = (it * kWaves + wave) * 16 + jn, pos = pu < P ? pu : P - 1;
            const int f = pos - (pos / kFw) * kFw;
            const bool lok = f != 0, rok = f != kFw - 1;
            const char* xb = Hb + (pos * 4 + g) * 4;
            v4f d = cb[od];
#pragma unroll
            for (int kk = 0; kk < 6; ++kk) {
                const int o = kk >> 1;
                float x = *reinterpret_cast<const float*>(xb + ((2 + (kk & 1)) * kPmax + (o - 1)) * 16);
                if (o == 0) x = lok ? x : 0.0f;
                if (o == 2) x = rok ? x : 0.0f;
                d = mfma16x16x4(wa[od][kk], x, d);
            }
            const v2f d0 = mk2(d[0], d[1]), d1 = mk2(d[2], d[3]);
            const v2f a0 = d0 * mk2(pw1_slope, pw1_slope), a1 = d1 * mk2(pw1_slope, pw1_slope);
            const float4 r4 = make_float4(prelu_m(d0[0], a0[0], pw1_sel), prelu_m(d0[1], a0[1], pw1_sel),
                                          prelu_m(d1[0], a1[0], pw1_sel), prelu_m(d1[1], a1[1], pw1_sel));
            const bool now = (g < 2) != (od != 0);
            if (now && pu < P) H[(g & 1) * kPmax + pu] = r4;
            if (!od) {
                hi[it >> 1] = r4;
            } else {
                hi[it >> 1] = make_float4(now ? hi[it >> 1].x : r4.x, now ? hi[it >> 1].y : r4.y, now ? hi[it >> 1].z : r4.z, now ? hi[it >> 1].w : r4.w);
            }
        }
    }
    __syncthreads();
#pragma unroll
    for (int pr = 0; pr < kPairs; ++pr) {
        const int it = 2 * pr + (g < 2 ? 1 : 0);
        const int pu = (it * kWaves + wave) * 16 + jn;
        if (it < kTiles && pu < P) H[(2 + (g & 1)) * kPmax + pu] = hi[pr];
    }
    if (tid < 12) zt[tid] = 0.0f;
    if (sg.prev && tid == 0) xwait(sg.fi + kXFlagHist + blk, sg.err, xcode(kXFlagHist + blk));
    __syncthreads();
    ADE_CLK(1);

    float4 h1r[kPairs];
    {
        v2f wd[3][3][2];
#pragma unroll
        for (int kt = 0; kt < 3; ++kt)
#pragma unroll
            for (int kf = 0; kf < 3; ++kf) {
                const int o = kt * 48 + kf * 16 + 4 * g;
                wd[kt][kf][0] = mk2(c_dw[o], c_dw[o + 1]);
                wd[kt][kf][1] = mk2(c_dw[o + 2], c_dw[o + 3]);
            }
        const v2f db0 = mk2(c_dw_b[4 * g], c_dw_b[4 * g + 1]), db1 = mk2(c_dw_b[4 * g + 2], c_dw_b[4 * g + 3]);
        const int dstep = dilation * kFw * 16;
        const char* const zp = Hb + kZ0;
        auto dw_taps = [&](v2f& acc0, v2f& acc1, const int tj, const int f, const int prow, const int nkt) {
            const bool lok = f != 0, rok = f != kFw - 1;
            const char* const rb = Hb + ((g * kPmax + prow) * 16 - 16);
#pragma unroll
            for (int kt = 0; kt < 3; ++kt) {
                if (kt >= nkt) continue;
                const int src = tj - (2 - kt) * dilation;
                const bool tv = nkt == 3 ? (kt == 2 ? true : prow >= (2 - kt) * dilation * kFw) : (src >= 0 && src < T);
                const char* const row = tv ? rb - (2 - kt) * dstep : zp;
                const char* const la = lok ? row : zp;
                const char* const ra = rok ? row : zp;
                const float4 x0 = *reinterpret_cast<const float4*>(la);
                const float4 x1 = *reinterpret_cast<const float4*>(row + 16);
                const float4 x2 = *reinterpret_cast<const float4*>(ra + 32);
                acc0 += wd[kt][0][0] * mk2(x0.x, x0.y);
                acc1 += wd[kt][0][1] * mk2(x0.z, x0.w);
                acc0 += wd[kt][1][0] * mk2(x1.x, x1.y);
                acc1 += wd[kt][1][1] * mk2(x1.z, x1.w);
                acc0 += wd[kt][2][0] * mk2(x2.x, x2.y);
                acc1 += wd[kt][2][1] * mk2(x2.z, x2.w);
            }
        };
        float* const xhist_o = sg.xo + blk * kXHistFloats;
        const float* const xhist_i = sg.xi + blk * kXHistFloats;
        const int NP = 2 * dilation * kFw;
        if (sg.next) {
#pragma unroll 1
            for (int pt = wave; pt * 16 < NP; pt += kWaves) {
                const int pu = pt * 16 + jn, pn = pu < NP ? pu : NP - 1;
                const int tn = pn / kFw, f = pn - tn * kFw;
                const int j = tn + T;
                v2f acc0 = db0, acc1 = db1;
                if (sg.prev && j < 2 * dilation) {
                    const float4 v = xld4(xhist_i, (g * kXHistFrames * kFw + j * kFw + f) * 4);
                    acc0 = mk2(v.x, v.y);
                    acc1 = mk2(v.z, v.w);
                }
                dw_taps(acc0, acc1, j, f, pn + P, 2);
                if (pu < NP) xst4(xhist_o, (g * kXHistFrames * kFw + pn) * 4, make_float4(acc0[0], acc0[1], acc1[0], acc1[1]));
            }
            xdrain();
            __syncthreads();
            if (tid == 0) xflag_store(sg.fo + kXFlagHist + blk, 1u);
        }
        float wp[2][4];
#pragma unroll
        for (int r = 0; r < 4; ++r) {
            const float wv = c_pw2[(4 * g + r) * 8 + (jn & 7)];
            wp[0][r] = jn < 8 ? wv : 0.0f;
            wp[1][r] = jn < 8 ? 0.0f : wv;
        }
        v4f cb2;
#pragma unroll
        for (int r = 0; r < 4; ++r) cb2[r] = c_pw2_b[(4 * g + r) & 7];
        v4f d2 = cb2;
#pragma unroll
        for (int it = 0; it < kTiles; ++it) {
            const int pu = (it * kWaves + wave) * 16 + jn, pos = pu < P ? pu : P - 1;
            const int t = pos / kFw, f = pos - t * kFw;
            v2f acc0 = db0, acc1 = db1;
            if (sg.prev && (it * kWaves + wave) * 16 < NP) {
                const float4 v = xld4(xhist_i, (g * kXHistFrames * kFw + (pos < NP ? pos : NP - 1)) * 4);
                const bool head = pos < NP;
                acc0 = mk2(head ? v.x : db0[0], head ? v.y : db0[1]);
                acc1 = mk2(head ? v.z : db1[0], head ? v.w : db1[1]);
            }
            dw_taps(acc0, acc1, t, f, pos, 3);
            const v2f a0 = acc0 * mk2(dw_slope, dw_slope), a1 = acc1 * mk2(dw_slope, dw_slope);
            const float y[4] = {prelu_m(acc0[0], a0[0], dw_sel), prelu_m(acc0[1], a0[1], dw_sel),
                                prelu_m(acc1[0], a1[0], dw_sel), prelu_m(acc1[1], a1[1], dw_sel)};
            if (!(it & 1)) d2 = cb2;
#pragma unroll
            for (int r = 0; r < 4; ++r) d2 = mfma16x16x4(wp[it & 1][r], y[r], d2);
            if ((it & 1) || it == kTiles - 1) h1r[it >> 1] = make_float4(d2[0], d2[1], d2[2], d2[3]);
        }
    }
    __syncthreads();
    ADE_CLK(2);
#pragma unroll
    for (int pr = 0; pr < kPairs; ++pr) {
        const int it = 2 * pr + (g >> 1);
        const int pu = (it * kWaves + wave) * 16 + jn;
        if (it < kTiles && pu < P) H[(g & 1) * kPmax + pu] = h1r[pr];
    }
    __syncthreads();
    ADE_CLK(3);

    v2f wr_raw[8];
    float bh_raw = 0.0f;
    {
        const int j = tid & 15, row = (tid >> 4) & 3;
        const int gsel = (row & 1) ? 2 : (row >> 1);
        const float* pk = w.gru + j * 78 + 24 + gsel * 16;
#pragma unroll
        for (int m = 0; m < 8; ++m) wr_raw[m] = tid < 64 ? mk2(pk[2 * m], pk[2 * m + 1]) : mk2(0.0f, 0.0f);
        if (tid < 64) bh_raw = w.gru[j * 78 + 75 + gsel];
    }
    const float* nsc = (next_x1 && next_skip) ? next_skip + cbase : nullptr;
    float nsk[kPosPerThread][8];
    auto request_next_skip = [&]() {
#pragma unroll
        for (int i = 0; i < kPosPerThread; ++i) {
            const int p = tid + i * kFusedThreads;
            if (nsc && p < P) {
                pl_ld8(nsc, Ps, p, 0, nsk[i]);
            } else {
#pragma unroll
                for (int k = 0; k < 8; ++k) nsk[i][k] = 0.0f;
            }
        }
    };
    request_next_skip();
    {
        const int tr = tid >> 4, j = tid & 15;
        const int t = tr < T ? tr : T - 1;
        {
            float e[8] = {0.0f, 0.0f, 0.0f, 0.0f, 0.0f, 0.0f, 0.0f, 0.0f};
#pragma unroll
            for (int u = 0; u < 3; ++u) {
                const int f = j + 16 * u;
                if (f < kFw) {
                    const float4 a0 = H[t * kFw + f], a1 = H[kPmax + t * kFw + f];
                    e[0] += a0.x * a0.x; e[1] += a0.y * a0.y; e[2] += a0.z * a0.z; e[3] += a0.w * a0.w;
                    e[4] += a1.x * a1.x; e[5] += a1.y * a1.y; e[6] += a1.z * a1.z; e[7] += a1.w * a1.w;
                }
            }
#pragma unroll
            for (int c = 0; c < 8; ++c) {
                e[c] += row_ror<8>(e[c]);
                e[c] += row_ror<4>(e[c]);
                e[c] += row_ror<2>(e[c]);
                e[c] += row_ror<1>(e[c]);
                e[c] = e[c] * (1.0f / (float)kFw);
            }
            const float* pk = w.gru + j * 78;
#pragma unroll
            for (int g = 0; g < 3; ++g) {
                float sacc = pk[72 + g];
#pragma unroll
                for (int k = 0; k < 8; ++k) sacc += pk[g * 8 + k] * e[k];
                if (tr < T) GI[t * 48 + g * 16 + j] = sacc * (g == 2 ? 2.0f * kLog2e : -kLog2e);
            }
        }
    }
    if (sg.prev && tid == 0) xwait(sg.fi + kXFlagTra + blk, sg.err, xcode(kXFlagTra + blk));
    __syncthreads();
    ADE_CLK(4);
    ADE_CLK(5);
    if (tid >= 64) {
        constexpr int kLanes = kFusedThreads - 64, kIt = (kPmax + kLanes - 1) / kLanes;
        float by[kIt][8], y[kIt][8];
#pragma unroll
        for (int i = 0; i < kIt; ++i) {
            const int p = tid - 64 + i * kLanes, pc = p < P ? p : P - 1;
            pl_ld8(ac, Ps, pc, 2, by[i]);
            if (sc) pl_ld8(sc, Ps, pc, 2, y[i]);
        }
#pragma unroll
        for (int i = 0; i < kIt; ++i) {
            const int p = tid - 64 + i * kLanes;
            if (p >= P) break;
            if (sc) {
#pragma unroll
                for (int k = 0; k < 8; ++k) by[i][k] += y[i][k];
            }
            H[p] = make_float4(by[i][0], by[i][1], by[i][2], by[i][3]);
            H[kPmax + p] = make_float4(by[i][4], by[i][5], by[i][6], by[i][7]);
        }
    } else {
        const int j = tid & 15, row = tid >> 4;
        const int gsel = (row & 1) ? 2 : (row >> 1);
        const float sc = gsel == 2 ? 2.0f * kLog2e : -kLog2e;
        v2f wr[8];
#pragma unroll
        for (int m = 0; m < 8; ++m) wr[m] = wr_raw[m] * sc;
        const float bh = bh_raw * sc;
        int shb[16];
        float hv = 0.0f;
        if (sg.prev) hv = xld1(sg.xi + kXTraOff + blk * 16 + j);
#define ADE_RL(K) shb[K] = __builtin_amdgcn_readlane(__float_as_int(hv), K);
        ADE_REP16(ADE_RL)
#undef ADE_RL
        float gi = GI[gsel * 16 + j];
        float* hsp = row == 3 ? HS + j : GI + (tid & 63);
        const int hs_step = row == 3 ? 16 : 0;
        __builtin_amdgcn_s_setprio(3);
        for (int t = 0; t < T; ++t) {
            const int tn = t + 1 < T ? t + 1 : t;
            const float gnx = GI[tn * 48 + gsel * 16 + j];
#pragma unroll
            for (int k = 0; k < 16; ++k) ADE_KEEP_IN_LOOP(shb[k]);
            float sh[16];
#pragma unroll
            for (int k = 0; k < 16; ++k) sh[k] = __int_as_float(shb[k]);
            v2f a0 = mk2(bh, 0.0f), a1 = mk2(0.0f, 0.0f);
#pragma unroll
            for (int m = 0; m < 8; m += 2) {
                a0 += wr[m] * mk2(sh[2 * m], sh[2 * m + 1]);
                a1 += wr[m + 1] * mk2(sh[2 * m + 2], sh[2 * m + 3]);
            }
            const v2f a2 = a0 + a1;
            const float a = a2[0] + a2[1];
            const float e = __builtin_amdgcn_exp2f(gi + a);
            const float sg = fast_rcp(1.0f + e);
            const float X = swap16(e, sg).a;
            const float en = __builtin_amdgcn_exp2f(gi + X * a);
            const float n = 1.0f - 2.0f * fast_rcp(en + 1.0f);
            const float n3 = swap32(en, n).a;
            const float hc = n3 + X * (hv - n3);
            hv = hc;
#define ADE_RL(K) shb[K] = __builtin_amdgcn_readlane(__float_as_int(hc), 48 + K);
            ADE_REP16(ADE_RL)
#undef ADE_RL
            *hsp = hc;
            hsp += hs_step;
            gi = gnx;
        }
        set_prio(sg.base_prio);
        if (sg.next) {
            if (row == 3) xst1(sg.xo + kXTraOff + blk * 16 + j, hv);
            xdrain();
            if (tid == 48) xflag_store(sg.fo + kXFlagTra + blk, 1u);
        }
    }
    __syncthreads();
    ADE_CLK(6);
    for (int idx = tid; idx < T * 8; idx += kFusedThreads) {
        const int t = idx >> 3, c = idx & 7;
        const float* fr = w.fc + c * 17;
        float s = fr[16];
#pragma unroll
        for (int k = 0; k < 16; ++k) s += fr[k] * HS[t * 16 + k];
        at[idx] = sigmoid_f(s);
    }
    __syncthreads();
    ADE_CLK(7);
#pragma unroll
    for (int pr = 0; pr < kPairs; ++pr) {
        const int it = 2 * pr + (g >> 1);
        const int pu = (it * kWaves + wave) * 16 + jn;
        if (it < kTiles && pu < P) {
            const float4 gt = *reinterpret_cast<const float4*>(at + (pu / kFw) * 8 + 4 * (g & 1));
            H[(2 + (g & 1)) * kPmax + pu] = make_float4(h1r[pr].x * gt.x, h1r[pr].y * gt.y, h1r[pr].z * gt.z, h1r[pr].w * gt.w);
        }
    }
    __syncthreads();
    float n8[kPosPerThread][8];
#pragma unroll
    for (int i = 0; i < kPosPerThread; ++i) {
        const int p = tid + i * kFusedThreads;
        if (p < P) {
            const float4 b0 = H[p], b1 = H[kPmax + p], g0 = H[2 * kPmax + p], g1 = H[3 * kPmax + p];
            const float o[16] = {g0.x, b0.x, g0.y, b0.y, g0.z, b0.z, g0.w, b0.w, g1.x, b1.x, g1.y, b1.y, g1.z, b1.z, g1.w, b1.w};
            if (store_lo) {
                pl_st16(oc, Ps, p, o);
            } else {
                st4(oc + ((size_t)2 * Ps + p) * 4, o + 8);
                st4(oc + ((size_t)3 * Ps + p) * 4, o + 12);
            }
#pragma unroll
            for (int k = 0; k < 8; ++k) n8[i][k] = o[k] + nsk[i][k];
            if (next_full) {
#pragma unroll
                for (int q = 0; q < 4; ++q) H[q * kPmax + p] = make_float4(o[4 * q], o[4 * q + 1], o[4 * q + 2], o[4 * q + 3]);
            }
        }
    }
    if (next_x1) {
        __syncthreads();
#pragma unroll
        for (int i = 0; i < kPosPerThread; ++i) {
            const int p = tid + i * kFusedThreads;
            if (p < P) {
                H[2 * kPmax + p] = make_float4(n8[i][0], n8[i][1], n8[i][2], n8[i][3]);
                H[3 * kPmax + p] = make_float4(n8[i][4], n8[i][5], n8[i][6], n8[i][7]);
            }
        }
    }
    ADE_CLK(8);
}

template <class G> constexpr size_t dp_smem_bytes() { return (size_t)4 * G::kPmax * 16 + (size_t)2 * kFw * kCh * 4; }

template <class G, class EmitPos, class EmitOne>
__device__ __forceinline__ void fc_ln_rows(float4* R, const float* __restrict__ fc, const float* __restrict__ fc_b, const float* __restrict__ ln_w,
                                           const float* __restrict__ ln_b, int T, int P, int tid, const float* __restrict__ res, int Ps, EmitPos emit_pos, EmitOne emit_one) {
    constexpr int kFusedThreads = G::kThreads, kPmax = G::kPmax;
    static_assert(kFusedThreads / 16 >= G::kTmax, "one 16-lane row per frame");
    {
        constexpr int kWaves = kFusedThreads / 64, kTiles = (kPmax / 16 + kWaves - 1) / kWaves;
        int tq = tid;
        ADE_OPAQUE_V(tq);
        const int wave = __builtin_amdgcn_readfirstlane(tq >> 6), g = (tq >> 4) & 3, jn = tq & 15;
        float wa[4];
#pragma unroll
        for (int kk = 0; kk < 4; ++kk) wa[kk] = fc[(4 * g + kk) * 16 + jn];
        v4f cb;
#pragma unroll
        for (int r = 0; r < 4; ++r) cb[r] = fc_b[4 * g + r];
#pragma unroll
        for (int it = 0; it < kTiles; ++it) {
            const int pu = (it * kWaves + wave) * 16 + jn, pos = pu < P ? pu : P - 1;
            const float4 x = R[g * kPmax + pos];
            v4f d = cb;
            d = mfma16x16x4(wa[0], x.x, d);
            d = mfma16x16x4(wa[1], x.y, d);
            d = mfma16x16x4(wa[2], x.z, d);
            d = mfma16x16x4(wa[3], x.w, d);
            if (pu < P) R[g * kPmax + pu] = make_float4(d[0], d[1], d[2], d[3]);
        }
    }
    __syncthreads();
    int tq = tid;
    ADE_OPAQUE_V(tq);
    const int tr = tq >> 4, j = tq & 15;
    const bool live = tr < T;
    const int t = live ? tr : T - 1;
    const int p0 = t * kFw + j, p1 = p0 + 16, p2 = t * kFw + 32;
    float* Rf = reinterpret_cast<float*>(R);
    auto allreduce = [](float s) { s += row_ror<8>(s); s += row_ror<4>(s); s += row_ror<2>(s); s += row_ror<1>(s); return s; };
    float rs0[16], rs1[16];
    pl_ld16(res, Ps, p0, rs0);
    const float re = res[((size_t)(j >> 2) * Ps + p2) * 4 + (j & 3)];
    float v0[16], v1[16];
#pragma unroll
    for (int q = 0; q < 4; ++q) {
        const float4 a = R[q * kPmax + p0], b = R[q * kPmax + p1];
        v0[4 * q] = a.x; v0[4 * q + 1] = a.y; v0[4 * q + 2] = a.z; v0[4 * q + 3] = a.w;
        v1[4 * q] = b.x; v1[4 * q + 1] = b.y; v1[4 * q + 2] = b.z; v1[4 * q + 3] = b.w;
    }
    const float e = Rf[((size_t)(j >> 2) * kPmax + p2) * 4 + (j & 3)];
    float s = e;
#pragma unroll
    for (int c = 0; c < 16; ++c) s += v0[c] + v1[c];
    const float mean = allreduce(s) * (1.0f / (float)(kFw * kCh));
    const float de = e - mean;
    float q2 = de * de;
#pragma unroll
    for (int c = 0; c < 16; ++c) { const float a = v0[c] - mean, b = v1[c] - mean; q2 += a * a + b * b; }
    const float rstd = fast_rsq(allreduce(q2) * (1.0f / (float)(kFw * kCh)) + 1e-8f);
    {
        float gw[16], gb[16];
        ld16(ln_w + j * kCh, gw);
        ld16(ln_b + j * kCh, gb);
#pragma unroll
        for (int c = 0; c < 16; ++c) v0[c] = ((v0[c] - mean) * rstd * gw[c] + gb[c]) + rs0[c];
        if (live) emit_pos(p0, v0);
    }
    {
        float gw[16], gb[16];
        pl_ld16(res, Ps, p1, rs1);
        ld16(ln_w + (16 + j) * kCh, gw);
        ld16(ln_b + (16 + j) * kCh, gb);
#pragma unroll
        for (int c = 0; c < 16; ++c) v1[c] = ((v1[c] - mean) * rstd * gw[c] + gb[c]) + rs1[c];
        if (live) emit_pos(p1, v1);
    }
    {
        const float ye = (de * rstd * ln_w[32 * kCh + j] + ln_b[32 * kCh + j]) + re;
        if (live) emit_one(p2, j, ye);
    }
}

__device__ __forceinline__ float gru_gates(const v4f& d, float h) {
    const float r = fast_rcp(1.0f + __builtin_amdgcn_exp2f(d[0]));
    const float z = fast_rcp(1.0f + __builtin_amdgcn_exp2f(d[1]));
    const float n = 1.0f - 2.0f * fast_rcp(__builtin_amdgcn_exp2f(d[3] + r * d[2]) + 1.0f);
    return n + z * (h - n);
}

template <class G>
__device__ __forceinline__ void dpgrnn_stage(float4* smem, int chunk, const Seg& sg, int blk, const float* __restrict__ x, const DpW& w, float* __restrict__ out,
                                             long long* __restrict__ clk, bool next_x1 = false,
                                             const float* __restrict__ next_skip = nullptr, bool store_lo = true, bool x_in_lds = false, bool next_full = false) {
    constexpr int kFusedThreads = G::kThreads, kTmaxFused = G::kTmax, kPmax = G::kPmax, kPosPerThread = G::kPosPerThread;
    float4* R = smem;
    float* Rf = reinterpret_cast<float*>(smem);
    float* lnt = reinterpret_cast<float*>(smem + 4 * kPmax);
    const int T = sg.nT;
    const int P = T * kFw, Ps = sg.T * kFw;
    int tid_ = threadIdx.x;
    ADE_OPAQUE_V(tid_);
    const int tid = tid_;
    for (int i = tid; i < kFw * kCh; i += kFusedThreads) {
        lnt[i] = w.intra_ln_w[i];
        lnt[kFw * kCh + i] = w.intra_ln_b[i];
    }
    const size_t cbase = (size_t)chunk * kCh * Ps + (size_t)sg.t0 * kFw * 4;
    const float* xc = x + cbase;
    float* oc = out + cbase;

    ADE_CLK(16);
    {
        constexpr float kS = -kLog2e, kN = 2.0f * kLog2e;
        if (!x_in_lds) {
            float4 v[kPosPerThread][4];
#pragma unroll
            for (int i = 0; i < kPosPerThread; ++i) {
                const int p = tid + i * kFusedThreads, pc = p < P ? p : P - 1;
#pragma unroll
                for (int q = 0; q < 4; ++q) v[i][q] = *reinterpret_cast<const float4*>(xc + ((size_t)q * Ps + pc) * 4);
            }
#pragma unroll
            for (int i = 0; i < kPosPerThread; ++i) {
                const int p = tid + i * kFusedThreads;
                if (p < P) {
#pragma unroll
                    for (int q = 0; q < 4; ++q) R[q * kPmax + p] = v[i][q];
                }
            }
            __syncthreads();
        }
        const int wave = __builtin_amdgcn_readfirstlane(tid >> 6);
        const int g = (tid >> 4) & 3, j = tid & 15;
        const int grp = (wave >> 1) & 1, dir = wave & 1, t = (wave >> 2) * 16 + j;
        const bool live = t < T;
        const int tc = live ? t : T - 1;
        float ax0, ax1, ah;
        {
            const int c = j & 3;
            const float* pk = w.intra_gru + (grp * 8 + dir * 4 + (j >> 2)) * 42;
            const float sc_ = c < 2 ? kS : kN;
            const int gi = c == 3 ? 2 : c;
            ax0 = c == 2 ? 0.0f : pk[gi * 8 + g] * sc_;
            ax1 = c == 2 ? 0.0f : pk[gi * 8 + 4 + g] * sc_;
            ah = c == 3 ? 0.0f : pk[24 + c * 4 + g] * sc_;
        }
        v4f cb;
        {
            const float* pb = w.intra_gru + (grp * 8 + dir * 4 + g) * 42;
            cb[0] = (pb[36] + pb[39]) * kS;
            cb[1] = (pb[37] + pb[40]) * kS;
            cb[2] = pb[41] * kN;
            cb[3] = pb[38] * kN;
        }
        const float* const xr = Rf + ((size_t)(grp * 2) * kPmax + tc * kFw) * 4 + g;
        float hout[kFw];
        auto run = [&](auto dir_c) {
            constexpr int DIR = decltype(dir_c)::value;
            float h = 0.0f;
            __builtin_amdgcn_s_setprio(3);
            v4f dx;
            {
                constexpr int f0 = DIR ? kFw - 1 : 0;
                dx = mfma16x16x4(ax0, xr[f0 * 4], cb);
                dx = mfma16x16x4(ax1, xr[(kPmax + f0) * 4], dx);
            }
#pragma unroll
            for (int s = 0; s < kFw; ++s) {
                v4f d = mfma16x16x4(ah, h, dx);
                if (s + 1 < kFw) {
                    const int fn = DIR ? kFw - 2 - s : s + 1;
                    dx = mfma16x16x4(ax0, xr[fn * 4], cb);
                    dx = mfma16x16x4(ax1, xr[(kPmax + fn) * 4], dx);
                }
                h = gru_gates(d, h);
                hout[s] = h;
            }
            set_prio(sg.base_prio);
            __syncthreads();
            float* const hw = Rf + ((size_t)(grp * 2 + DIR) * kPmax + tc * kFw) * 4 + g;
            if (live) {
#pragma unroll
                for (int s = 0; s < kFw; ++s) hw[(DIR ? kFw - 1 - s : s) * 4] = hout[s];
            }
        };
        if (dir) run(std::integral_constant<int, 1>{});
        else run(std::integral_constant<int, 0>{});
    }
    __syncthreads();
    ADE_CLK(17);
    fc_ln_rows<G>(R, w.intra_fc, w.intra_fc_b, lnt, lnt + kFw * kCh, T, P, tid, xc, Ps,
        [&](int p, const float (&m)[16]) {
#pragma unroll
            for (int q = 0; q < 4; ++q) R[q * kPmax + p] = make_float4(m[4 * q], m[4 * q + 1], m[4 * q + 2], m[4 * q + 3]);
            pl_st16(oc, Ps, p, m);
        },
        [&](int p, int c, float m) {
            Rf[((size_t)(c >> 2) * kPmax + p) * 4 + (c & 3)] = m;
            oc[((size_t)(c >> 2) * Ps + p) * 4 + (c & 3)] = m;
        });
    if (sg.prev && tid == 0) xwait(sg.fi + kXFlagInter + blk, sg.err, xcode(kXFlagInter + blk));
    __syncthreads();
    for (int i = tid; i < kFw * kCh; i += kFusedThreads) {
        lnt[i] = w.inter_ln_w[i];
        lnt[kFw * kCh + i] = w.inter_ln_b[i];
    }
    ADE_CLK(18);
#if ADE_DP_INTER_MFMA
    {
        constexpr float kS = -kLog2e, kN = 2.0f * kLog2e;
        constexpr int kWaves = kFusedThreads / 64, kTilesC = 6;
        static_assert(kWaves % 2 == 0, "a wavefront's tiles share its group");
        const int wave = __builtin_amdgcn_readfirstlane(tid >> 6);
        const int g = (tid >> 4) & 3, j = tid & 15;
        const int grp = wave & 1;
        float ax[2][2], ah[2][2];
        v4f cb[2];
#pragma unroll
        for (int U = 0; U < 2; ++U) {
            const int c = j & 3;
            const float* pk = w.inter_gru + (grp * 8 + 4 * U + (j >> 2)) * 54;
            const float sc_ = c < 2 ? kS : kN;
            const int gi = c == 3 ? 2 : c;
#pragma unroll
            for (int kk = 0; kk < 2; ++kk) {
                ax[U][kk] = c == 2 ? 0.0f : pk[gi * 8 + 4 * kk + g] * sc_;
                ah[U][kk] = c == 3 ? 0.0f : pk[24 + c * 8 + 4 * kk + g] * sc_;
            }
            const float* pb = w.inter_gru + (grp * 8 + 4 * U + g) * 54;
            cb[U][0] = (pb[48] + pb[51]) * kS;
            cb[U][1] = (pb[49] + pb[52]) * kS;
            cb[U][2] = pb[53] * kN;
            cb[U][3] = pb[50] * kN;
        }
        auto run = [&](auto nt_c) {
            constexpr int NT = decltype(nt_c)::value;
            float h[NT][2];
            bool live[NT];
            float* xp[NT];
            float* xs[NT];
            v4f dx[NT][2];
#pragma unroll
            for (int c = 0; c < NT; ++c) {
                const int tile = wave + c * kWaves, f = (tile >> 1) * 16 + j;
                live[c] = f < kFw;
                const int fc = live[c] ? f : kFw - 1;
                xp[c] = Rf + ((size_t)(grp * 2) * kPmax + fc) * 4 + g;
                xs[c] = sg.xi + kXInterOff + blk * (kFw * 16) + fc * 16 + grp;
                h[c][0] = h[c][1] = 0.0f;
                if (sg.prev) {
                    h[c][0] = xld1(xs[c] + 2 * g);
                    h[c][1] = xld1(xs[c] + 2 * (4 + g));
                }
                const float x0 = xp[c][0], x1 = xp[c][kPmax * 4];
#pragma unroll
                for (int U = 0; U < 2; ++U) {
                    dx[c][U] = mfma16x16x4(ax[U][0], x0, cb[U]);
                    dx[c][U] = mfma16x16x4(ax[U][1], x1, dx[c][U]);
                }
            }
            __builtin_amdgcn_s_setprio(3);
            for (int t = 0; t < T; ++t) {
                const int tn = t + 1 < T ? 1 : 0;
#pragma unroll
                for (int c = 0; c < NT; ++c) {
                    v4f d[2];
#pragma unroll
                    for (int U = 0; U < 2; ++U) {
                        d[U] = mfma16x16x4(ah[U][0], h[c][0], dx[c][U]);
                        d[U] = mfma16x16x4(ah[U][1], h[c][1], d[U]);
                    }
                    float* const xn = xp[c] + tn * (kFw * 4);
                    const float x0 = xn[0], x1 = xn[kPmax * 4];
#pragma unroll
                    for (int U = 0; U < 2; ++U) {
                        dx[c][U] = mfma16x16x4(ax[U][0], x0, cb[U]);
                        dx[c][U] = mfma16x16x4(ax[U][1], x1, dx[c][U]);
                    }
                    h[c][0] = gru_gates(d[0], h[c][0]);
                    h[c][1] = gru_gates(d[1], h[c][1]);
                    if (live[c]) {
                        xp[c][0] = h[c][0];
                        xp[c][kPmax * 4] = h[c][1];
                    }
                    xp[c] = xn;
                }
            }
            set_prio(sg.base_prio);
            if (sg.next) {
#pragma unroll
                for (int c = 0; c < NT; ++c) {
                    float* const xo = sg.xo + (xs[c] - sg.xi);
                    if (live[c]) {
                        xst1(xo + 2 * g, h[c][0]);
                        xst1(xo + 2 * (4 + g), h[c][1]);
                    }
                }
                xdrain();
            }
        };
        const int nt = wave < kTilesC ? (kTilesC - 1 - wave) / kWaves + 1 : 0;
        static_assert((kTilesC + kWaves - 1) / kWaves <= 2, "at most two tiles per wavefront");
        if (nt == 2) run(std::integral_constant<int, 2>{});
        else if (nt == 1) run(std::integral_constant<int, 1>{});
    }
#else
    {
        constexpr int kRows = G::kThreads / 16;
        const int row = tid >> 4, q = tid & 15;
        const int grp = q & 1, unit = q >> 1;
        const float* pk = w.inter_gru + (grp * 8 + unit) * 54;
        int ks[8];
        ks[0] = unit;
#define ADE_KS(S) ks[S] = ((int)row_ror<2 * S>((float)q)) >> 1;
        ADE_KS(1) ADE_KS(2) ADE_KS(3) ADE_KS(4) ADE_KS(5) ADE_KS(6) ADE_KS(7)
#undef ADE_KS
        constexpr float kS = -kLog2e, kN = 2.0f * kLog2e;
        v2f wi_rz[8], wh_rz[8], wi_n[4], wh_n[4];
#pragma unroll
        for (int k = 0; k < 8; ++k) {
            wi_rz[k] = mk2(pk[k] * kS, pk[8 + k] * kS);
            wh_rz[k] = mk2(pk[24 + ks[k]] * kS, pk[32 + ks[k]] * kS);
        }
#pragma unroll
        for (int m = 0; m < 4; ++m) {
            wi_n[m] = mk2(pk[16 + 2 * m] * kN, pk[16 + 2 * m + 1] * kN);
            wh_n[m] = mk2(pk[40 + ks[2 * m]] * kN, pk[40 + ks[2 * m + 1]] * kN);
        }
        const v2f b_rz = mk2((pk[48] + pk[51]) * kS, (pk[49] + pk[52]) * kS);
        const float bi_n = pk[50] * kN, bh_n = pk[53] * kN;
        auto run = [&](auto nc_c) {
            constexpr int NC = decltype(nc_c)::value;
            float h[NC];
            float4 xa[NC], xb[NC];
            int fc_[NC];
            bool live[NC];
#pragma unroll
            for (int c = 0; c < NC; ++c) {
                const int f = row + kRows * c;
                live[c] = f < kFw;
                fc_[c] = live[c] ? f : kFw - 1;
                h[c] = 0.0f;
                if (sg.prev) h[c] = xld1(sg.xi + kXInterOff + blk * (kFw * 16) + fc_[c] * 16 + q);
                xa[c] = R[(grp * 2) * kPmax + fc_[c]];
                xb[c] = R[(grp * 2 + 1) * kPmax + fc_[c]];
            }
            __builtin_amdgcn_s_setprio(3);
            for (int t = 0; t < T; ++t) {
                const int tn = t + 1 < T ? t + 1 : t;
#pragma unroll
                for (int c = 0; c < NC; ++c) {
                    const int p = t * kFw + fc_[c], pn = tn * kFw + fc_[c];
                    const float xv[8] = {xa[c].x, xa[c].y, xa[c].z, xa[c].w, xb[c].x, xb[c].y, xb[c].z, xb[c].w};
                    xa[c] = R[(grp * 2) * kPmax + pn];
                    xb[c] = R[(grp * 2 + 1) * kPmax + pn];
                    v2f a_rz = b_rz, a_n = mk2(bi_n, 0.0f);
#pragma unroll
                    for (int k = 0; k < 8; ++k) a_rz += wi_rz[k] * xv[k];
#pragma unroll
                    for (int m = 0; m < 4; ++m) a_n += wi_n[m] * mk2(xv[2 * m], xv[2 * m + 1]);
                    float hs[8];
                    hs[0] = h[c];
#define ADE_HS(S) hs[S] = row_ror<2 * S>(h[c]);
                    ADE_HS(1) ADE_HS(2) ADE_HS(3) ADE_HS(4) ADE_HS(5) ADE_HS(6) ADE_HS(7)
#undef ADE_HS
                    v2f c0 = a_rz, c1 = mk2(0.0f, 0.0f), c_n = mk2(bh_n, 0.0f);
#pragma unroll
                    for (int k = 0; k < 8; k += 2) { c0 += wh_rz[k] * hs[k]; c1 += wh_rz[k + 1] * hs[k + 1]; }
#pragma unroll
                    for (int m = 0; m < 4; ++m) c_n += wh_n[m] * mk2(hs[2 * m], hs[2 * m + 1]);
                    const v2f rz = c0 + c1;
                    const float r = fast_rcp(1.0f + __builtin_amdgcn_exp2f(rz[0]));
                    const float z = fast_rcp(1.0f + __builtin_amdgcn_exp2f(rz[1]));
                    const float n = 1.0f - 2.0f * fast_rcp(__builtin_amdgcn_exp2f((a_n[0] + a_n[1]) + r * (c_n[0] + c_n[1])) + 1.0f);
                    h[c] = n + z * (h[c] - n);
                    if (live[c]) Rf[((size_t)(grp * 2 + (unit >> 2)) * kPmax + p) * 4 + (unit & 3)] = h[c];
                }
            }
            set_prio(sg.base_prio);
            if (sg.next) {
#pragma unroll
                for (int c = 0; c < NC; ++c)
                    if (live[c]) xst1(sg.xo + kXInterOff + blk * (kFw * 16) + fc_[c] * 16 + q, h[c]);
                xdrain();
            }
        };
        const int row0 = (tid >> 6) * 4, nc = row0 < kFw ? (kFw - 1 - row0) / kRows + 1 : 0;
        static_assert((kFw + kRows - 1) / kRows <= 3, "at most three columns per 16-lane row");
        if (nc == 3) run(std::integral_constant<int, 3>{});
        else if (nc == 2) run(std::integral_constant<int, 2>{});
        else if (nc == 1) run(std::integral_constant<int, 1>{});
    }
#endif
    __syncthreads();
    if (sg.next && tid == 0) xflag_store(sg.fo + kXFlagInter + blk, 1u);
    ADE_CLK(19);
    {
        const float* nsc = (next_x1 && next_skip) ? next_skip + cbase : nullptr;
        fc_ln_rows<G>(R, w.inter_fc, w.inter_fc_b, lnt, lnt + kFw * kCh, T, P, tid, oc, Ps,
            [&](int p, const float (&o)[16]) {
                if (store_lo) {
                    pl_st16(oc, Ps, p, o);
                } else {
                    st4(oc + ((size_t)2 * Ps + p) * 4, o + 8);
                    st4(oc + ((size_t)3 * Ps + p) * 4, o + 12);
                }
                if (next_full) {
#pragma unroll
                    for (int q = 0; q < 4; ++q) R[q * kPmax + p] = make_float4(o[4 * q], o[4 * q + 1], o[4 * q + 2], o[4 * q + 3]);
                }
                if (next_x1) {
                    float k8[8] = {0.0f, 0.0f, 0.0f, 0.0f, 0.0f, 0.0f, 0.0f, 0.0f};
                    if (nsc) pl_ld8(nsc, Ps, p, 0, k8);
                    R[2 * kPmax + p] = make_float4(o[0] + k8[0], o[1] + k8[1], o[2] + k8[2], o[3] + k8[3]);
                    R[3 * kPmax + p] = make_float4(o[4] + k8[4], o[5] + k8[5], o[6] + k8[6], o[7] + k8[7]);
                }
            },
            [&](int p, int c, float o) {
                if (store_lo || c >= 8) oc[((size_t)(c >> 2) * Ps + p) * 4 + (c & 3)] = o;
                if (next_full) Rf[((size_t)(c >> 2) * kPmax + p) * 4 + (c & 3)] = o;
                if (next_x1 && c < 8) {
                    const float k = nsc ? nsc[((size_t)(c >> 2) * Ps + p) * 4 + (c & 3)] : 0.0f;
                    Rf[((size_t)(2 + (c >> 2)) * kPmax + p) * 4 + (c & 3)] = o + k;
                }
            });
    }
    ADE_CLK(20);
}


}
}
```

Before: 761,100 audio-s/s.

## Route global loads and stores through scalar buffer resources with split offsets

Replaces raw pointer accesses to global activations, PCM and exchange buffers across the frontend, backend and net stages with AMD buffer load/store intrinsics. Base addresses go into a wave-uniform resource descriptor via readfirstlane, and offsets are split into 32-bit vector and scalar parts. This is meant to cut 64-bit address arithmetic and VGPR pressure in the fused kernel. The exchange accessors move from atomic loads/stores to buffer ops with a cache-policy bit, and a guard is added that disables the fused path when the input is too large for 32-bit offsets. The lean-mode LDS placement of window sums and pending data is also changed.

Result: no change. 757,200 audio-s/s (-0.5%).

```diff
diff --git a/audio_denoiser_onnx_amd/csrc/ade_device.h b/audio_denoiser_onnx_amd/csrc/ade_device.h
--- a/audio_denoiser_onnx_amd/csrc/ade_device.h
+++ b/audio_denoiser_onnx_amd/csrc/ade_device.h
@@ -184,27 +184,79 @@
 
 #if defined(__AMDGCN__)
 typedef unsigned ade_v4u __attribute__((ext_vector_type(4)));
-__device__ __forceinline__ float4 xld4(const float* base, int float_off) {
-    const __amdgpu_buffer_rsrc_t r = __builtin_amdgcn_make_buffer_rsrc(const_cast<float*>(base), 0, 0x7fffffff, 0x00020000);
-    const ade_v4u v = __builtin_amdgcn_raw_buffer_load_b128(r, float_off * 4, 0, 16);
+typedef unsigned ade_v2u __attribute__((ext_vector_type(2)));
+struct GView { __amdgpu_buffer_rsrc_t r; };
+__device__ __forceinline__ GView gview(const void* base) {
+    const unsigned long long a = reinterpret_cast<unsigned long long>(base);
+    const unsigned lo = __builtin_amdgcn_readfirstlane((unsigned)a), hi = __builtin_amdgcn_readfirstlane((unsigned)(a >> 32));
+    GView v;
+    v.r = __builtin_amdgcn_make_buffer_rsrc(reinterpret_cast<void*>(((unsigned long long)hi << 32) | lo), 0, 0x7fffffff, 0x00020000);
+    return v;
+}
+template <int AUX = 0> __device__ __forceinline__ float4 gld16(const GView& g, unsigned voff, unsigned soff = 0) {
+    const ade_v4u v = __builtin_amdgcn_raw_buffer_load_b128(g.r, voff, soff, AUX);
     return make_float4(__int_as_float((int)v.x), __int_as_float((int)v.y), __int_as_float((int)v.z), __int_as_float((int)v.w));
 }
-__device__ __forceinline__ void xst4(float* base, int float_off, const float4& v) {
-    const __amdgpu_buffer_rsrc_t r = __builtin_amdgcn_make_buffer_rsrc(base, 0, 0x7fffffff, 0x00020000);
+template <int AUX = 0> __device__ __forceinline__ int4 gld16i(const GView& g, unsigned voff, unsigned soff = 0) {
+    const ade_v4u v = __builtin_amdgcn_raw_buffer_load_b128(g.r, voff, soff, AUX);
+    return make_int4((int)v.x, (int)v.y, (int)v.z, (int)v.w);
+}
+template <int AUX = 0> __device__ __forceinline__ float gld4(const GView& g, unsigned voff, unsigned soff = 0) {
+    return __int_as_float((int)__builtin_amdgcn_raw_buffer_load_b32(g.r, voff, soff, AUX));
+}
+template <int AUX = 0> __device__ __forceinline__ int gld4i(const GView& g, unsigned voff, unsigned soff = 0) {
+    return (int)__builtin_amdgcn_raw_buffer_load_b32(g.r, voff, soff, AUX);
+}
+template <int AUX = 0> __device__ __forceinline__ int gld2s(const GView& g, unsigned voff, unsigned soff = 0) {
+    return (int)(short)__builtin_amdgcn_raw_buffer_load_b16(g.r, voff, soff, AUX);
+}
+template <int AUX = 0> __device__ __forceinline__ void gst16(const GView& g, unsigned voff, unsigned soff, const float4& v) {
     ade_v4u u;
     u.x = (unsigned)__float_as_int(v.x); u.y = (unsigned)__float_as_int(v.y); u.z = (unsigned)__float_as_int(v.z); u.w = (unsigned)__float_as_int(v.w);
-    __builtin_amdgcn_raw_buffer_store_b128(u, r, float_off * 4, 0, 16);
-}
-__device__ __forceinline__ float xld1(const float* p) { return __hip_atomic_load(p, __ATOMIC_RELAXED, __HIP_MEMORY_SCOPE_AGENT); }
-__device__ __forceinline__ void xst1(float* p, float v) { __hip_atomic_store(p, v, __ATOMIC_RELAXED, __HIP_MEMORY_SCOPE_AGENT); }
+    __builtin_amdgcn_raw_buffer_store_b128(u, g.r, voff, soff, AUX);
+}
+template <int AUX = 0> __device__ __forceinline__ void gst8(const GView& g, unsigned voff, unsigned soff, const float2& v) {
+    ade_v2u u;
+    u.x = (unsigned)__float_as_int(v.x); u.y = (unsigned)__float_as_int(v.y);
+    __builtin_amdgcn_raw_buffer_store_b64(u, g.r, voff, soff, AUX);
+}
+template <int AUX = 0> __device__ __forceinline__ void gst8s(const GView& g, unsigned voff, unsigned soff, const short4& v) {
+    ade_v2u u;
+    u.x = ((unsigned)(unsigned short)v.x) | ((unsigned)(unsigned short)v.y << 16);
+    u.y = ((unsigned)(unsigned short)v.z) | ((unsigned)(unsigned short)v.w << 16);
+    __builtin_amdgcn_raw_buffer_store_b64(u, g.r, voff, soff, AUX);
+}
+template <int AUX = 0> __device__ __forceinline__ void gst4(const GView& g, unsigned voff, unsigned soff, float v) {
+    __builtin_amdgcn_raw_buffer_store_b32((unsigned)__float_as_int(v), g.r, voff, soff, AUX);
+}
+#else
+struct GView { char* b; };
+__device__ __forceinline__ GView gview(const void* base) { return GView{const_cast<char*>(reinterpret_cast<const char*>(base))}; }
+template <int AUX = 0> __device__ __forceinline__ float4 gld16(const GView& g, unsigned voff, unsigned soff = 0) { return *reinterpret_cast<const float4*>(g.b + voff + soff); }
+template <int AUX = 0> __device__ __forceinline__ int4 gld16i(const GView& g, unsigned voff, unsigned soff = 0) { return *reinterpret_cast<const int4*>(g.b + voff + soff); }
+template <int AUX = 0> __device__ __forceinline__ float gld4(const GView& g, unsigned voff, unsigned soff = 0) { return *reinterpret_cast<const float*>(g.b + voff + soff); }
+template <int AUX = 0> __device__ __forceinline__ int gld4i(const GView& g, unsigned voff, unsigned soff = 0) { return *reinterpret_cast<const int*>(g.b + voff + soff); }
+template <int AUX = 0> __device__ __forceinline__ int gld2s(const GView& g, unsigned voff, unsigned soff = 0) { return (int)*reinterpret_cast<const int16_t*>(g.b + voff + soff); }
+template <int AUX = 0> __device__ __forceinline__ void gst16(const GView& g, unsigned voff, unsigned soff, const float4& v) { *reinterpret_cast<float4*>(g.b + voff + soff) = v; }
+template <int AUX = 0> __device__ __forceinline__ void gst8(const GView& g, unsigned voff, unsigned soff, const float2& v) { *reinterpret_cast<float2*>(g.b + voff + soff) = v; }
+template <int AUX = 0> __device__ __forceinline__ void gst8s(const GView& g, unsigned voff, unsigned soff, const short4& v) { *reinterpret_cast<short4*>(g.b + voff + soff) = v; }
+template <int AUX = 0> __device__ __forceinline__ void gst4(const GView& g, unsigned voff, unsigned soff, float v) { *reinterpret_cast<float*>(g.b + voff + soff) = v; }
+#endif
+__device__ __forceinline__ void gld16v(const GView& g, unsigned voff, unsigned soff, float* v) {
+    const float4 q = gld16(g, voff, soff);
+    v[0] = q.x; v[1] = q.y; v[2] = q.z; v[3] = q.w;
+}
+__device__ __forceinline__ void gst16v(const GView& g, unsigned voff, unsigned soff, const float* v) { gst16(g, voff, soff, make_float4(v[0], v[1], v[2], v[3])); }
+
+__device__ __forceinline__ float4 xld4(const GView& x, int float_off) { return gld16<16>(x, (unsigned)float_off * 4u); }
+__device__ __forceinline__ void xst4(const GView& x, int float_off, const float4& v) { gst16<16>(x, (unsigned)float_off * 4u, 0, v); }
+__device__ __forceinline__ float xld1(const GView& x, int float_off) { return gld4<16>(x, (unsigned)float_off * 4u); }
+__device__ __forceinline__ void xst1(const GView& x, int float_off, float v) { gst4<16>(x, (unsigned)float_off * 4u, 0, v); }
+#if defined(__AMDGCN__)
 __device__ __forceinline__ unsigned xflag_load(const unsigned* p) { return __hip_atomic_load(p, __ATOMIC_RELAXED, __HIP_MEMORY_SCOPE_AGENT); }
 __device__ __forceinline__ void xflag_store(unsigned* p, unsigned v) { __hip_atomic_store(p, v, __ATOMIC_RELAXED, __HIP_MEMORY_SCOPE_AGENT); }
 __device__ __forceinline__ void xdrain() { asm volatile("s_waitcnt vmcnt(0)" ::: "memory"); }
 #else
-__device__ __forceinline__ float4 xld4(const float* base, int float_off) { return *reinterpret_cast<const float4*>(base + float_off); }
-__device__ __forceinline__ void xst4(float* base, int float_off, const float4& v) { *reinterpret_cast<float4*>(base + float_off) = v; }
-__device__ __forceinline__ float xld1(const float* p) { return *p; }
-__device__ __forceinline__ void xst1(float* p, float v) { *p = v; }
 __device__ __forceinline__ unsigned xflag_load(const unsigned* p) { return *(const volatile unsigned*)p; }
 __device__ __forceinline__ void xflag_store(unsigned* p, unsigned v) { *(volatile unsigned*)p = v; }
 __device__ __forceinline__ void xdrain() {}
diff --git a/audio_denoiser_onnx_amd/csrc/ade_engine.hip b/audio_denoiser_onnx_amd/csrc/ade_engine.hip
--- a/audio_denoiser_onnx_amd/csrc/ade_engine.hip
+++ b/audio_denoiser_onnx_amd/csrc/ade_engine.hip
@@ -637,6 +637,7 @@
 };
 
 int pick_geometry(const ade_engine* e, int ) {
+    if ((long long)e->in_len * (long long)sizeof(int16_t) >= (1ll << 31)) return -1;
     if (e->geometry >= 0) return fused_supported(e->T, e->geometry) ? e->geometry : -1;
     for (int g = fused_geometries() - 1; g >= 0; --g)
         if (fused_supported(e->T, g)) return g;
diff --git a/audio_denoiser_onnx_amd/csrc/ade_stage_frontback.h b/audio_denoiser_onnx_amd/csrc/ade_stage_frontback.h
--- a/audio_denoiser_onnx_amd/csrc/ade_stage_frontback.h
+++ b/audio_denoiser_onnx_amd/csrc/ade_stage_frontback.h
@@ -28,7 +28,7 @@
     return LdsTabs{win, reinterpret_cast<const float2*>(tw256), reinterpret_cast<const float2*>(tw512)};
 }
 
-__device__ __forceinline__ void load_frame_pairs(const int16_t* __restrict__ row, int L, int t, int lane, bool live, bool pair_ok, int* raw, int centre = kNfft / 2) {
+__device__ __forceinline__ void load_frame_pairs(const GView& row, int L, int t, int lane, bool live, bool pair_ok, int* raw, int centre = kNfft / 2) {
 #pragma unroll
     for (int r = 0; r < 4; ++r) {
         const int n = lane + 64 * r;
@@ -36,16 +36,29 @@
         if (!live) {
             raw[r] = 0;
         } else if (pair_ok && j0 >= 0 && j0 + 1 < L) {
-            raw[r] = *reinterpret_cast<const int*>(row + j0);
+            raw[r] = gld4i(row, (unsigned)j0 * 2u);
         } else {
             int ja = j0, jb = j0 + 1;
             ja = ja < 0 ? -ja : (ja >= L ? 2 * (L - 1) - ja : ja);
             jb = jb < 0 ? -jb : (jb >= L ? 2 * (L - 1) - jb : jb);
-            raw[r] = ((int)row[ja] & 0xffff) | ((int)row[jb] << 16);
-        }
-    }
-}
-
+            raw[r] = (gld2s(row, (unsigned)ja * 2u) & 0xffff) | (gld2s(row, (unsigned)jb * 2u) << 16);
+        }
+    }
+}
+
+__device__ __forceinline__ void erb_merge(const GView& wtab, int count, int s0, const float2* buf, int lane, float* fr) {
+    float a0 = 0.0f, a1 = 0.0f, a2 = 0.0f;
+    for (int n = 0; n < count; ++n) {
+        const float wv = gld4(wtab, (unsigned)lane * 4u, (unsigned)n * (kErbBands * 4u));
+        const float2 x = buf[kErbLow + min(s0 + n, kErbHigh - 1)];
+        a0 += fast_sqrt((x.x * x.x + x.y * x.y) + 1e-12f) * wv;
+        a1 += x.x * wv;
+        a2 += x.y * wv;
+    }
+    fr[kErbLow + lane] = a0;
+    fr[kErb + kErbLow + lane] = a1;
+    fr[2 * kErb + kErbLow + lane] = a2;
+}
 __device__ __forceinline__ void erb_merge(const float* wtab, int count, int s0, const float2* buf, int lane, float* fr) {
     float a0 = 0.0f, a1 = 0.0f, a2 = 0.0f;
     for (int n = 0; n < count; ++n) {
@@ -90,13 +103,15 @@
     int tid_ = threadIdx.x;
     ADE_OPAQUE_V(tid_);
     const int tid = tid_, wave = tid >> 6, lane = tid & 63;
-    const int16_t* row = pcm + (size_t)chunk * L;
+    const int16_t* const rowp = pcm + (size_t)chunk * L;
+    const GView row = gview(rowp);
     const int P0 = T * kF1, P = T * kFw;
-    float* e0c = e0 + (size_t)chunk * kCh * P0;
-    float* e1c = e1 + (size_t)chunk * kCh * P;
-    float* specc = spec + (size_t)chunk * T * 2 * kBinsPad;
+    const GView e0c = gview(e0 + (size_t)chunk * kCh * P0);
+    const GView e1c = gview(e1 + (size_t)chunk * kCh * P);
+    const GView specc = gview(spec + (size_t)chunk * T * 2 * kBinsPad);
+    const GView erbv = gview(erb.w);
     ADE_CLK(32);
-    const bool pair_ok = ((L & 1) == 0) && ((reinterpret_cast<size_t>(row) & 3) == 0);
+    const bool pair_ok = ((L & 1) == 0) && ((reinterpret_cast<size_t>(rowp) & 3) == 0);
     int raw[4];
     const int centre = sg.stream ? 0 : kNfft / 2;
     load_frame_pairs(row, L, tbeg + wave, lane, tbeg + wave < tend, pair_ok, raw, centre);
@@ -111,16 +126,15 @@
 
     if (!dc_rows) {
         int s = 0;
-        if (((L & 7) == 0) && ((reinterpret_cast<size_t>(row) & 15) == 0)) {
-            const int4* r4 = reinterpret_cast<const int4*>(row);
+        if (((L & 7) == 0) && ((reinterpret_cast<size_t>(rowp) & 15) == 0)) {
 #pragma unroll 2
             for (int i = tid; i < (L >> 3); i += kFusedThreads) {
-                const int4 q = r4[i];
+                const int4 q = gld16i(row, (unsigned)i * 16u);
                 s += (int)(short)(q.x & 0xffff) + (q.x >> 16) + (int)(short)(q.y & 0xffff) + (q.y >> 16)
                    + (int)(short)(q.z & 0xffff) + (q.z >> 16) + (int)(short)(q.w & 0xffff) + (q.w >> 16);
             }
         } else {
-            for (int i = tid; i < L; i += kFusedThreads) s += (int)row[i];
+            for (int i = tid; i < L; i += kFusedThreads) s += gld2s(row, (unsigned)i * 2u);
         }
 #pragma unroll
         for (int off = 32; off >= 1; off >>= 1) s += __shfl_xor(s, off);
@@ -195,8 +209,8 @@
                     if (r == 4 && lane != 0) break;
                     const int k = r < 4 ? lane + 64 * r : 256;
                     const float2 x = buf[k];
-                    specc[((size_t)t * 2 + 0) * kBinsPad + k] = x.x;
-                    specc[((size_t)t * 2 + 1) * kBinsPad + k] = x.y;
+                    gst4(specc, (unsigned)((t * 2 + 0) * kBinsPad + k) * 4u, 0, x.x);
+                    gst4(specc, (unsigned)((t * 2 + 1) * kBinsPad + k) * 4u, 0, x.y);
                     if (k < kErbLow) {
                         fr[k] = fast_sqrt((x.x * x.x + x.y * x.y) + 1e-12f);
                         fr[kErb + k] = x.x;
@@ -204,7 +218,7 @@
                     }
                 }
                 if (erb_lds) erb_merge(erbw, erb.count, erb_s0, buf, lane, fr);
-                else erb_merge(erb.w, erb.count, erb_s0, buf, lane, fr);
+                else erb_merge(erbv, erb.count, erb_s0, buf, lane, fr);
             }
         }
         __syncthreads();
@@ -241,7 +255,7 @@
                                                   prelu_m(d[2], d[2] * c0.slope, sel0), prelu_m(d[3], d[3] * c0.slope, sel0));
                     const int idx = tl * kF1 + fo;
                     E0[g * kTileP1 + idx] = r4;
-                    *reinterpret_cast<float4*>(e0c + ((size_t)g * P0 + (size_t)t0 * kF1 + idx) * 4) = r4;
+                    gst16(e0c, (unsigned)(t0 * kF1 + idx) * 16u, (unsigned)(g * P0) * 16u, r4);
                 }
             }
         }
@@ -265,7 +279,7 @@
                 acc = prelu_f(acc, c0.slope);
                 const int idx = tl * kF1 + (kF1 - 1);
                 E0f[((size_t)(co >> 2) * kTileP1 + idx) * 4 + (co & 3)] = acc;
-                e0c[((size_t)(co >> 2) * P0 + t0 * kF1 + idx) * 4 + (co & 3)] = acc;
+                gst4(e0c, pl_elem(co, P0, t0 * kF1 + idx), 0, acc);
             }
         }
         __syncthreads();
@@ -298,8 +312,8 @@
 #pragma unroll
                 for (int co = 0; co < 8; ++co) acc[co] = prelu_f(acc[co], c1.slope);
                 const int p = t0 * kFw + tl * kFw + fo;
-                st4(e1c + ((size_t)(2 * g) * P + p) * 4, acc);
-                st4(e1c + ((size_t)(2 * g + 1) * P + p) * 4, acc + 4);
+                gst16v(e1c, pl_pos(p), pl_plane(2 * g, P), acc);
+                gst16v(e1c, pl_pos(p), pl_plane(2 * g + 1, P), acc + 4);
             }
         }
         if (tid < kTileF * 16) {
@@ -317,7 +331,7 @@
                 }
                 acc = prelu_f(acc, c1.slope);
                 const int p = t0 * kFw + tl * kFw + (kFw - 1);
-                e1c[((size_t)(2 * g + (co >> 2)) * P + p) * 4 + (co & 3)] = acc;
+                gst4(e1c, pl_elem(8 * g + co, P, p), 0, acc);
             }
         }
         ADE_CLK(36);
@@ -359,21 +373,34 @@
     float* bsw = tabmem + kTabFloats;
     float* w3t = bsw + kBsCap * kErbHigh;
     float* w4t = w3t + kC3TailW;
-    float* wsum = kLean ? const_cast<float*>(tabs.win_sum) : w4t + kC4TailW;
+    float* wsum = w4t + kC4TailW;
     int* bss = reinterpret_cast<int*>(wsum + kHop);
-    float* pend = kLean ? sg.xo + kXPendOff : reinterpret_cast<float*>(bss + kErbHigh);
+    float* pend = reinterpret_cast<float*>(bss + kErbHigh);
+    const GView wsumv = gview(tabs.win_sum), bssv = gview(bs.start);
+    const GView xi = gview(sg.xi), xo = gview(sg.xo);
     int tid_ = threadIdx.x;
     ADE_OPAQUE_V(tid_);
     const int tid = tid_;
     const int P0 = T * kF1, P = T * kFw;
-    const float* xc = x + (size_t)chunk * kCh * P;
-    const float* e1c = e1 + (size_t)chunk * kCh * P;
-    const float* e0c = e0 + (size_t)chunk * kCh * P0;
-    const float* specc = spec + (size_t)chunk * T * 2 * kBinsPad;
+    const GView xc = gview(x + (size_t)chunk * kCh * P);
+    const GView e1c = gview(e1 + (size_t)chunk * kCh * P);
+    const GView e0c = gview(e0 + (size_t)chunk * kCh * P0);
+    const GView specc = gview(spec + (size_t)chunk * T * 2 * kBinsPad);
     const int trim = sg.stream ? 0 : kHop;
     const int out_len = sg.stream ? kHop * T : kHop * (T - 1);
-    int16_t* po = pcm ? pcm + (size_t)chunk * out_len : nullptr;
-    float* fo32 = f32 ? f32 + (size_t)chunk * out_len : nullptr;
+    const bool po_on = pcm != nullptr, fo32_on = f32 != nullptr;
+    const GView po = gview(pcm + (po_on ? (size_t)chunk * out_len : 0));
+    const GView fo32 = gview(f32 + (fo32_on ? (size_t)chunk * out_len : 0));
+    auto ld_wsum = [&](int i, float* ws) { if (kLean) gld16v(wsumv, (unsigned)i * 4u, 0, ws); else ld4(wsum + i, ws); };
+    auto st_out = [&](int n, const float* v) {
+        if (fo32_on) gst16v(fo32, (unsigned)n * 4u, 0, v);
+        if (po_on) {
+            short q[4];
+#pragma unroll
+            for (int u = 0; u < 4; ++u) q[u] = (short)(int)fminf(fmaxf(v[u] * 32767.0f, -32768.0f), 32767.0f);
+            gst8s(po, (unsigned)n * 2u, 0, make_short4(q[0], q[1], q[2], q[3]));
+        }
+    };
     ADE_CLK(48);
 
     auto issue_s = [&](int t0n, bool go, float4* sa, float4* sb) {
@@ -385,9 +412,9 @@
         for (int i = 0; i < 3; ++i) {
             const int u = tq + kSThreads * i, q = u / kTileP, idx = u - q * kTileP;
             const int idc = idx < nfn * kFw ? idx : 0;
-            const size_t off = ((size_t)q * P + (size_t)t0n * kFw + idc) * 4;
-            sa[i] = on ? *reinterpret_cast<const float4*>(xc + off) : make_float4(0.0f, 0.0f, 0.0f, 0.0f);
-            sb[i] = on ? *reinterpret_cast<const float4*>(e1c + off) : make_float4(0.0f, 0.0f, 0.0f, 0.0f);
+            const unsigned off = (unsigned)(q * P + t0n * kFw + idc) * 16u;
+            sa[i] = on ? gld16(xc, off) : make_float4(0.0f, 0.0f, 0.0f, 0.0f);
+            sb[i] = on ? gld16(e1c, off) : make_float4(0.0f, 0.0f, 0.0f, 0.0f);
         }
     };
     auto commit_s = [&](const float4* sa, const float4* sb) {
@@ -408,9 +435,9 @@
         const int pe = on ? tl * kF1 + 2 * m : 0;
 #pragma unroll
         for (int h = 0; h < 2; ++h) {
-            const float* src = e0c + ((size_t)(2 * g + h) * P0 + (size_t)t0n * kF1 + pe) * 4;
-            ea[h] = on ? *reinterpret_cast<const float4*>(src) : make_float4(0.0f, 0.0f, 0.0f, 0.0f);
-            eb[h] = on ? *reinterpret_cast<const float4*>(src + 4) : make_float4(0.0f, 0.0f, 0.0f, 0.0f);
+            const unsigned src = (unsigned)((2 * g + h) * P0 + t0n * kF1 + pe) * 16u;
+            ea[h] = on ? gld16(e0c, src) : make_float4(0.0f, 0.0f, 0.0f, 0.0f);
+            eb[h] = on ? gld16(e0c, src + 16u) : make_float4(0.0f, 0.0f, 0.0f, 0.0f);
         }
     };
     float4 sa0[3], sb0[3];
@@ -433,7 +460,7 @@
 #pragma unroll
             for (int r = 1; r < 5; ++r) {
                 const int k = r < 4 ? lane + 64 * r : 256;
-                bs_s[r - 1] = (k >= kErbLow && (r < 4 || lane == 0)) ? bs.start[k - kErbLow] : 0;
+                bs_s[r - 1] = (k >= kErbLow && (r < 4 || lane == 0)) ? gld4i(bssv, (unsigned)(k - kErbLow) * 4u) : 0;
             }
         }
     }
@@ -449,7 +476,7 @@
         const int nf = tend - t0 < kTileF ? tend - t0 : kTileF;
         float sre[5], sim[5];
         float wsr[4] = {1.0f, 1.0f, 1.0f, 1.0f};
-        if (kLean) ld4(wsum + ((tid * 4) & (kHop - 1)), wsr);
+        if (kLean) ld_wsum((tid * 4) & (kHop - 1), wsr);
         {
             int tq = tid;
             ADE_OPAQUE_V(tq);
@@ -458,8 +485,8 @@
 #pragma unroll
             for (int r = 0; r < 5; ++r) {
                 const int k = r < 4 ? lane + 64 * r : 256;
-                sre[r] = (r < 4 || lane == 0) ? specc[((size_t)tcp * 2 + 0) * kBinsPad + k] : 0.0f;
-                sim[r] = (r < 4 || lane == 0) ? specc[((size_t)tcp * 2 + 1) * kBinsPad + k] : 0.0f;
+                sre[r] = (r < 4 || lane == 0) ? gld4(specc, (unsigned)((tcp * 2 + 0) * kBinsPad + k) * 4u) : 0.0f;
+                sim[r] = (r < 4 || lane == 0) ? gld4(specc, (unsigned)((tcp * 2 + 1) * kBinsPad + k) * 4u) : 0.0f;
             }
         }
         __syncthreads();
@@ -510,7 +537,7 @@
             const int tl = tq >> 4, g = (tq >> 3) & 1, co = tq & 7;
             if (tl < nf) {
                 const int pe = tl * kF1 + (kF1 - 1);
-                const float eadd = e0c[((size_t)(2 * g + (co >> 2)) * P0 + (size_t)t0 * kF1 + pe) * 4 + (co & 3)];
+                const float eadd = gld4(e0c, pl_elem(8 * g + co, P0, t0 * kF1 + pe));
                 float ev = b3t;
 #pragma unroll
                 for (int dlt = -1; dlt <= 0; ++dlt) {
@@ -643,7 +670,8 @@
                         ADE_OPAQUE_V(wb);
                         float2* a = reinterpret_cast<float2*>(acc + kHop * wave + 2 * n);
                         if (park && r < 2) {
-                            *reinterpret_cast<float2*>(pend + 2 * n) = make_float2(wa, wb);
+                            if (kLean) gst8(xo, (unsigned)(kXPendOff + 2 * n) * 4u, 0, make_float2(wa, wb));
+                            else *reinterpret_cast<float2*>(pend + 2 * n) = make_float2(wa, wb);
                         } else if (par == 0) {
                             float2 c = make_float2(0.0f, 0.0f);
                             if (wave == 0 && r < 2) c = *reinterpret_cast<const float2*>(cbuf + 2 * n);
@@ -678,19 +706,13 @@
             else ld4(wsum + (i & (kHop - 1)), ws);
 #pragma unroll
             for (int u = 0; u < 4; ++u) v[u] = v[u] * fast_rcp(ws[u]);
-            if (fo32) st4(fo32 + n, v);
-            if (po) {
-                short q[4];
-#pragma unroll
-                for (int u = 0; u < 4; ++u) q[u] = (short)(int)fminf(fmaxf(v[u] * 32767.0f, -32768.0f), 32767.0f);
-                *reinterpret_cast<short4*>(po + n) = make_short4(q[0], q[1], q[2], q[3]);
-            }
+            st_out(n, v);
         }
         ADE_CLK_ACC(60);
         {
             float carry = 0.0f;
             if (tf < kHop) carry = acc[kHop * nf + tf];
-            if (sg.next && !has_next && tf < kHop) xst1(sg.xo + kXOlaOff + tf, carry);
+            if (sg.next && !has_next && tf < kHop) xst1(xo, kXOlaOff + tf, carry);
             if (tf < kHop) cbuf[tf] = carry;
         }
         ADE_CLK_ACC(61);
@@ -709,17 +731,12 @@
             const int i = i4 * 4;
             const int n = kHop * tbeg + i - trim;
             float v[4], ws[4];
-            ld4(pend + i, v);
-            ld4(wsum + i, ws);
-#pragma unroll
-            for (int u = 0; u < 4; ++u) v[u] = (xld1(sg.xi + kXOlaOff + i + u) + v[u]) * fast_rcp(ws[u]);
-            if (fo32) st4(fo32 + n, v);
-            if (po) {
-                short q[4];
-#pragma unroll
-                for (int u = 0; u < 4; ++u) q[u] = (short)(int)fminf(fmaxf(v[u] * 32767.0f, -32768.0f), 32767.0f);
-                *reinterpret_cast<short4*>(po + n) = make_short4(q[0], q[1], q[2], q[3]);
-            }
+            if (kLean) gld16v(xo, (unsigned)(kXPendOff + i) * 4u, 0, v);
+            else ld4(pend + i, v);
+            ld_wsum(i, ws);
+#pragma unroll
+            for (int u = 0; u < 4; ++u) v[u] = (xld1(xi, kXOlaOff + i + u) + v[u]) * fast_rcp(ws[u]);
+            st_out(n, v);
         }
     }
     ADE_CLK(53);
diff --git a/audio_denoiser_onnx_amd/csrc/ade_stage_net.h b/audio_denoiser_onnx_amd/csrc/ade_stage_net.h
--- a/audio_denoiser_onnx_amd/csrc/ade_stage_net.h
+++ b/audio_denoiser_onnx_amd/csrc/ade_stage_net.h
@@ -32,18 +32,23 @@
 
 __device__ __forceinline__ float comp(const float4& v, int c) { return c == 0 ? v.x : (c == 1 ? v.y : (c == 2 ? v.z : v.w)); }
 
-__device__ __forceinline__ void pl_ld8(const float* Xc, int P, int p, int q0, float* v) {
-    ld4(Xc + ((size_t)q0 * P + p) * 4, v);
-    ld4(Xc + ((size_t)(q0 + 1) * P + p) * 4, v + 4);
+__device__ __forceinline__ unsigned pl_pos(int p) { return (unsigned)p * 16u; }
+__device__ __forceinline__ unsigned pl_plane(int q, int P) { return (unsigned)(q * P) * 16u; }
+__device__ __forceinline__ unsigned pl_elem(int c, int P, int p) { return (unsigned)(((c >> 2) * P + p) * 4 + (c & 3)) * 4u; }
+__device__ __forceinline__ void pl_ld8(const GView& Xc, int P, int p, int q0, float* v) {
+    gld16v(Xc, pl_pos(p), pl_plane(q0, P), v);
+    gld16v(Xc, pl_pos(p), pl_plane(q0 + 1, P), v + 4);
 }
-__device__ __forceinline__ void pl_ld16(const float* Xc, int P, int p, float* v) {
+__device__ __forceinline__ void pl_ld16(const GView& Xc, int P, int p, float* v) {
     pl_ld8(Xc, P, p, 0, v);
     pl_ld8(Xc, P, p, 2, v + 8);
 }
-__device__ __forceinline__ void pl_st16(float* Xc, int P, int p, const float* v) {
-#pragma unroll
-    for (int q = 0; q < 4; ++q) st4(Xc + ((size_t)q * P + p) * 4, v + 4 * q);
+__device__ __forceinline__ void pl_st16(const GView& Xc, int P, int p, const float* v) {
+#pragma unroll
+    for (int q = 0; q < 4; ++q) gst16v(Xc, pl_pos(p), pl_plane(q, P), v + 4 * q);
 }
+static_assert((long long)kMaxSegments * Geo0::kTmax * kF1 * kCh * 4 < (1ll << 31) && (long long)kMaxSegments * Geo0::kTmax * 2 * kBinsPad * 4 < (1ll << 31),
+              "per-chunk tensors must be addressable with 32-bit byte offsets");
 
 template <class G> constexpr size_t gt_smem_bytes() { return (size_t)4 * G::kPmax * 16 + 2 * G::kTmax * 8 * 4; }
 
@@ -72,9 +77,10 @@
     ADE_OPAQUE_V(tid_);
     const int tid = tid_;
     const size_t cbase = (size_t)chunk * kCh * Ps + (size_t)sg.t0 * kFw * 4;
-    const float* ac = a + cbase;
-    const float* sc = skip ? skip + cbase : nullptr;
-    float* oc = out + cbase;
+    const GView ac = gview(a + cbase), oc = gview(out + cbase);
+    const bool sc_on = skip != nullptr;
+    const GView sc = gview((sc_on ? skip : a) + cbase);
+    const GView xi = gview(sg.xi), xo = gview(sg.xo);
     const cfptr c_pw1_b = cptr(w.pw1_b), c_dw_b = cptr(w.dw_b), c_pw2_b = cptr(w.pw2_b);
     cfptr c_pw1, c_dw, c_pw2;
     ADE_SCALAR_COPY(c_pw1, cptr(w.pw1));
@@ -92,13 +98,13 @@
         for (int i = 0; i < kIt; ++i) {
             const int p = tid + i * kFusedThreads, pc = p < P ? p : P - 1;
             pl_ld8(ac, Ps, pc, 0, x[i]);
-            if (sc) pl_ld8(sc, Ps, pc, 0, y[i]);
+            if (sc_on) pl_ld8(sc, Ps, pc, 0, y[i]);
         }
 #pragma unroll
         for (int i = 0; i < kIt; ++i) {
             const int p = tid + i * kFusedThreads;
             if (p >= P) break;
-            if (sc) {
+            if (sc_on) {
 #pragma unroll
                 for (int k = 0; k < 8; ++k) x[i][k] += y[i][k];
             }
@@ -204,8 +210,7 @@
                 acc1 += wd[kt][2][1] * mk2(x2.z, x2.w);
             }
         };
-        float* const xhist_o = sg.xo + blk * kXHistFloats;
-        const float* const xhist_i = sg.xi + blk * kXHistFloats;
+        const int xhist = blk * kXHistFloats;
         const int NP = 2 * dilation * kFw;
         if (sg.next) {
 #pragma unroll 1
@@ -215,12 +220,12 @@
                 const int j = tn + T;
                 v2f acc0 = db0, acc1 = db1;
                 if (sg.prev && j < 2 * dilation) {
-                    const float4 v = xld4(xhist_i, (g * kXHistFrames * kFw + j * kFw + f) * 4);
+                    const float4 v = xld4(xi, xhist + (g * kXHistFrames * kFw + j * kFw + f) * 4);
                     acc0 = mk2(v.x, v.y);
                     acc1 = mk2(v.z, v.w);
                 }
                 dw_taps(acc0, acc1, j, f, pn + P, 2);
-                if (pu < NP) xst4(xhist_o, (g * kXHistFrames * kFw + pn) * 4, make_float4(acc0[0], acc0[1], acc1[0], acc1[1]));
+                if (pu < NP) xst4(xo, xhist + (g * kXHistFrames * kFw + pn) * 4, make_float4(acc0[0], acc0[1], acc1[0], acc1[1]));
             }
             xdrain();
             __syncthreads();
@@ -243,7 +248,7 @@
             const int t = pos / kFw, f = pos - t * kFw;
             v2f acc0 = db0, acc1 = db1;
             if (sg.prev && (it * kWaves + wave) * 16 < NP) {
-                const float4 v = xld4(xhist_i, (g * kXHistFrames * kFw + (pos < NP ? pos : NP - 1)) * 4);
+                const float4 v = xld4(xi, xhist + (g * kXHistFrames * kFw + (pos < NP ? pos : NP - 1)) * 4);
                 const bool head = pos < NP;
                 acc0 = mk2(head ? v.x : db0[0], head ? v.y : db0[1]);
                 acc1 = mk2(head ? v.z : db1[0], head ? v.w : db1[1]);
@@ -279,13 +284,14 @@
         for (int m = 0; m < 8; ++m) wr_raw[m] = tid < 64 ? mk2(pk[2 * m], pk[2 * m + 1]) : mk2(0.0f, 0.0f);
         if (tid < 64) bh_raw = w.gru[j * 78 + 75 + gsel];
     }
-    const float* nsc = (next_x1 && next_skip) ? next_skip + cbase : nullptr;
+    const bool nsc_on = next_x1 && next_skip;
+    const GView nsc = gview((nsc_on ? next_skip : a) + cbase);
     float nsk[kPosPerThread][8];
     auto request_next_skip = [&]() {
 #pragma unroll
         for (int i = 0; i < kPosPerThread; ++i) {
             const int p = tid + i * kFusedThreads;
-            if (nsc && p < P) {
+            if (nsc_on && p < P) {
                 pl_ld8(nsc, Ps, p, 0, nsk[i]);
             } else {
 #pragma unroll
@@ -337,13 +343,13 @@
         for (int i = 0; i < kIt; ++i) {
             const int p = tid - 64 + i * kLanes, pc = p < P ? p : P - 1;
             pl_ld8(ac, Ps, pc, 2, by[i]);
-            if (sc) pl_ld8(sc, Ps, pc, 2, y[i]);
+            if (sc_on) pl_ld8(sc, Ps, pc, 2, y[i]);
         }
 #pragma unroll
         for (int i = 0; i < kIt; ++i) {
             const int p = tid - 64 + i * kLanes;
             if (p >= P) break;
-            if (sc) {
+            if (sc_on) {
 #pragma unroll
                 for (int k = 0; k < 8; ++k) by[i][k] += y[i][k];
             }
@@ -360,7 +366,7 @@
         const float bh = bh_raw * sc;
         int shb[16];
         float hv = 0.0f;
-        if (sg.prev) hv = xld1(sg.xi + kXTraOff + blk * 16 + j);
+        if (sg.prev) hv = xld1(xi, kXTraOff + blk * 16 + j);
 #define ADE_RL(K) shb[K] = __builtin_amdgcn_readlane(__float_as_int(hv), K);
         ADE_REP16(ADE_RL)
 #undef ADE_RL
@@ -401,7 +407,7 @@
         }
         set_prio(sg.base_prio);
         if (sg.next) {
-            if (row == 3) xst1(sg.xo + kXTraOff + blk * 16 + j, hv);
+            if (row == 3) xst1(xo, kXTraOff + blk * 16 + j, hv);
             xdrain();
             if (tid == 48) xflag_store(sg.fo + kXFlagTra + blk, 1u);
         }
@@ -438,8 +444,8 @@
             if (store_lo) {
                 pl_st16(oc, Ps, p, o);
             } else {
-                st4(oc + ((size_t)2 * Ps + p) * 4, o + 8);
-                st4(oc + ((size_t)3 * Ps + p) * 4, o + 12);
+                gst16v(oc, pl_pos(p), pl_plane(2, Ps), o + 8);
+                gst16v(oc, pl_pos(p), pl_plane(3, Ps), o + 12);
             }
 #pragma unroll
             for (int k = 0; k < 8; ++k) n8[i][k] = o[k] + nsk[i][k];
@@ -467,7 +473,7 @@
 
 template <class G, class EmitPos, class EmitOne>
 __device__ __forceinline__ void fc_ln_rows(float4* R, const float* __restrict__ fc, const float* __restrict__ fc_b, const float* __restrict__ ln_w,
-                                           const float* __restrict__ ln_b, int T, int P, int tid, const float* __restrict__ res, int Ps, EmitPos emit_pos, EmitOne emit_one) {
+                                           const float* __restrict__ ln_b, int T, int P, int tid, const GView& res, int Ps, EmitPos emit_pos, EmitOne emit_one) {
     constexpr int kFusedThreads = G::kThreads, kPmax = G::kPmax;
     static_assert(kFusedThreads / 16 >= G::kTmax, "one 16-lane row per frame");
     {
@@ -504,7 +510,7 @@
     auto allreduce = [](float s) { s += row_ror<8>(s); s += row_ror<4>(s); s += row_ror<2>(s); s += row_ror<1>(s); return s; };
     float rs0[16], rs1[16];
     pl_ld16(res, Ps, p0, rs0);
-    const float re = res[((size_t)(j >> 2) * Ps + p2) * 4 + (j & 3)];
+    const float re = gld4(res, pl_elem(j, Ps, p2));
     float v0[16], v1[16];
 #pragma unroll
     for (int q = 0; q < 4; ++q) {
@@ -570,8 +576,8 @@
         lnt[kFw * kCh + i] = w.intra_ln_b[i];
     }
     const size_t cbase = (size_t)chunk * kCh * Ps + (size_t)sg.t0 * kFw * 4;
-    const float* xc = x + cbase;
-    float* oc = out + cbase;
+    const GView xc = gview(x + cbase), oc = gview(out + cbase);
+    const GView xi = gview(sg.xi), xo = gview(sg.xo);
 
     ADE_CLK(16);
     {
@@ -582,7 +588,7 @@
             for (int i = 0; i < kPosPerThread; ++i) {
                 const int p = tid + i * kFusedThreads, pc = p < P ? p : P - 1;
 #pragma unroll
-                for (int q = 0; q < 4; ++q) v[i][q] = *reinterpret_cast<const float4*>(xc + ((size_t)q * Ps + pc) * 4);
+                for (int q = 0; q < 4; ++q) v[i][q] = gld16(xc, pl_pos(pc), pl_plane(q, Ps));
             }
 #pragma unroll
             for (int i = 0; i < kPosPerThread; ++i) {
@@ -661,7 +667,7 @@
         },
         [&](int p, int c, float m) {
             Rf[((size_t)(c >> 2) * kPmax + p) * 4 + (c & 3)] = m;
-            oc[((size_t)(c >> 2) * Ps + p) * 4 + (c & 3)] = m;
+            gst4(oc, pl_elem(c, Ps, p), 0, m);
         });
     if (sg.prev && tid == 0) xwait(sg.fi + kXFlagInter + blk, sg.err, xcode(kXFlagInter + blk));
     __syncthreads();
@@ -702,7 +708,7 @@
             float h[NT][2];
             bool live[NT];
             float* xp[NT];
-            float* xs[NT];
+            int xs[NT];
             v4f dx[NT][2];
 #pragma unroll
             for (int c = 0; c < NT; ++c) {
@@ -710,11 +716,11 @@
                 live[c] = f < kFw;
                 const int fc = live[c] ? f : kFw - 1;
                 xp[c] = Rf + ((size_t)(grp * 2) * kPmax + fc) * 4 + g;
-                xs[c] = sg.xi + kXInterOff + blk * (kFw * 16) + fc * 16 + grp;
+                xs[c] = kXInterOff + blk * (kFw * 16) + fc * 16 + grp;
                 h[c][0] = h[c][1] = 0.0f;
                 if (sg.prev) {
-                    h[c][0] = xld1(xs[c] + 2 * g);
-                    h[c][1] = xld1(xs[c] + 2 * (4 + g));
+                    h[c][0] = xld1(xi, xs[c] + 2 * g);
+                    h[c][1] = xld1(xi, xs[c] + 2 * (4 + g));
                 }
                 const float x0 = xp[c][0], x1 = xp[c][kPmax * 4];
 #pragma unroll
@@ -754,10 +760,9 @@
             if (sg.next) {
 #pragma unroll
                 for (int c = 0; c < NT; ++c) {
-                    float* const xo = sg.xo + (xs[c] - sg.xi);
                     if (live[c]) {
-                        xst1(xo + 2 * g, h[c][0]);
-                        xst1(xo + 2 * (4 + g), h[c][1]);
+                        xst1(xo, xs[c] + 2 * g, h[c][0]);
+                        xst1(xo, xs[c] + 2 * (4 + g), h[c][1]);
                     }
                 }
                 xdrain();
@@ -805,7 +810,7 @@
                 live[c] = f < kFw;
                 fc_[c] = live[c] ? f : kFw - 1;
                 h[c] = 0.0f;
-                if (sg.prev) h[c] = xld1(sg.xi + kXInterOff + blk * (kFw * 16) + fc_[c] * 16 + q);
+                if (sg.prev) h[c] = xld1(xi, kXInterOff + blk * (kFw * 16) + fc_[c] * 16 + q);
                 xa[c] = R[(grp * 2) * kPmax + fc_[c]];
                 xb[c] = R[(grp * 2 + 1) * kPmax + fc_[c]];
             }
@@ -845,7 +850,7 @@
             if (sg.next) {
 #pragma unroll
                 for (int c = 0; c < NC; ++c)
-                    if (live[c]) xst1(sg.xo + kXInterOff + blk * (kFw * 16) + fc_[c] * 16 + q, h[c]);
+                    if (live[c]) xst1(xo, kXInterOff + blk * (kFw * 16) + fc_[c] * 16 + q, h[c]);
                 xdrain();
             }
         };
@@ -860,14 +865,15 @@
     if (sg.next && tid == 0) xflag_store(sg.fo + kXFlagInter + blk, 1u);
     ADE_CLK(19);
     {
-        const float* nsc = (next_x1 && next_skip) ? next_skip + cbase : nullptr;
+        const bool nsc_on = next_x1 && next_skip;
+        const GView nsc = gview((nsc_on ? next_skip : x) + cbase);
         fc_ln_rows<G>(R, w.inter_fc, w.inter_fc_b, lnt, lnt + kFw * kCh, T, P, tid, oc, Ps,
             [&](int p, const float (&o)[16]) {
                 if (store_lo) {
                     pl_st16(oc, Ps, p, o);
                 } else {
-                    st4(oc + ((size_t)2 * Ps + p) * 4, o + 8);
-                    st4(oc + ((size_t)3 * Ps + p) * 4, o + 12);
+                    gst16v(oc, pl_pos(p), pl_plane(2, Ps), o + 8);
+                    gst16v(oc, pl_pos(p), pl_plane(3, Ps), o + 12);
                 }
                 if (next_full) {
 #pragma unroll
@@ -875,16 +881,16 @@
                 }
                 if (next_x1) {
                     float k8[8] = {0.0f, 0.0f, 0.0f, 0.0f, 0.0f, 0.0f, 0.0f, 0.0f};
-                    if (nsc) pl_ld8(nsc, Ps, p, 0, k8);
+                    if (nsc_on) pl_ld8(nsc, Ps, p, 0, k8);
                     R[2 * kPmax + p] = make_float4(o[0] + k8[0], o[1] + k8[1], o[2] + k8[2], o[3] + k8[3]);
                     R[3 * kPmax + p] = make_float4(o[4] + k8[4], o[5] + k8[5], o[6] + k8[6], o[7] + k8[7]);
                 }
             },
             [&](int p, int c, float o) {
-                if (store_lo || c >= 8) oc[((size_t)(c >> 2) * Ps + p) * 4 + (c & 3)] = o;
+                if (store_lo || c >= 8) gst4(oc, pl_elem(c, Ps, p), 0, o);
                 if (next_full) Rf[((size_t)(c >> 2) * kPmax + p) * 4 + (c & 3)] = o;
                 if (next_x1 && c < 8) {
-                    const float k = nsc ? nsc[((size_t)(c >> 2) * Ps + p) * 4 + (c & 3)] : 0.0f;
+                    const float k = nsc_on ? gld4(nsc, pl_elem(c, Ps, p)) : 0.0f;
                     Rf[((size_t)(2 + (c >> 2)) * kPmax + p) * 4 + (c & 3)] = o + k;
                 }
             });
```
